# HuiyangYu/TGSFilter

Hardware: AMD Instinct MI355X
Metric: filtered Gbases/sec (end-to-end, excl. gzip I/O) (higher is better)
Workload: dtype u8

## Files before the change

include/tgsf_text.h:

```cpp
#ifndef TGSF_TEXT_H
#define TGSF_TEXT_H

#include "tgsf.h"

#ifdef __cplusplus
extern "C" {
#endif

#define TGSF_TEXT_ABI_VERSION 1
#define TGSF_TEXT_PAD 64u

enum {
    TGSF_TEXT_END = 0,
    TGSF_TEXT_IRREGULAR = 1,
    TGSF_TEXT_CAPACITY = 2
};

typedef struct tgsf_text_summary {
    uint32_t n_records;
    uint32_t stop;
    uint64_t consumed;
    uint64_t bases;
    uint32_t longest;
    float    device_ms;
} tgsf_text_summary;

typedef struct tgsf_text_index_arrays {
    uint64_t* seq_off;
    uint64_t* qual_off;
    uint32_t* len;
    uint64_t* name_off;
    uint32_t* name_len;
} tgsf_text_index_arrays;

typedef struct tgsf_text_device_buffers {
    uint8_t* text;
    tgsf_text_index_arrays index;
    tgsf_text_summary* summary;
    uint64_t max_bytes;
    uint32_t max_records;
    uint32_t reserved;
} tgsf_text_device_buffers;

typedef struct tgsf_text tgsf_text;

int tgsf_text_abi_version(void);
const char* tgsf_text_backend(void);

int tgsf_text_create(int device, uint64_t max_bytes, uint32_t max_records, tgsf_text** out);
void tgsf_text_destroy(tgsf_text* tx);
const char* tgsf_text_last_error(tgsf_text* tx);
int tgsf_text_profile(tgsf_text* tx, int enable);
int tgsf_text_buffers(tgsf_text* tx, tgsf_text_device_buffers* out);

int tgsf_text_index(tgsf_text* tx, const uint8_t* text, uint64_t n_bytes, int fasta, int final,
                    const tgsf_text_index_arrays* out_index, tgsf_text_summary* out_summary);

int tgsf_text_upload(tgsf_text* tx, const uint8_t* text, uint64_t n_bytes);

int tgsf_text_index_device(tgsf_text* tx, const uint8_t* d_text, uint64_t n_bytes, int fasta, int final,
                           const tgsf_text_index_arrays* d_index, tgsf_text_summary* d_summary, void* hip_stream);

int tgsf_text_fetch(tgsf_text* tx, const tgsf_text_index_arrays* out_index, tgsf_text_summary* out_summary);

int tgsf_text_submit(tgsf_text* tx, tgsf_ctx* ctx, const uint8_t* text, uint64_t n_bytes, int fasta, int final,
                     const tgsf_text_index_arrays* out_index, tgsf_text_summary* out_summary, tgsf_batch_out* batch_out);

#ifdef __cplusplus
}
#endif
#endif
```

tgsfilter_amd/csrc/tgsf_text.hip:

```cpp
#include <stdarg.h>
#include <stdio.h>
#include <stdlib.h>
#include <string.h>

#include <algorithm>
#include <string>
#include <vector>

#if defined(TGSF_EMUL)
#include "tgsf_text_kernels.h"
namespace tgsf_emul { thread_local Dim3 threadIdx, blockIdx, blockDim, gridDim; }
typedef void* rt_stream;
#include "tgsf_emul_rt.h"
#else
#include <hip/hip_runtime.h>
#include "tgsf_text_kernels.h"
typedef hipStream_t rt_stream;
static int rt_malloc(void** p, size_t n) { return (int)hipMalloc(p, n ? n : 1); }
static void rt_free(void* p) { (void)hipFree(p); }
static int rt_memset(void* p, int v, size_t n, rt_stream s) { return (int)hipMemsetAsync(p, v, n, s); }
static int rt_h2d(void* d, const void* s, size_t n, rt_stream st) { return (int)hipMemcpyAsync(d, s, n, hipMemcpyHostToDevice, st); }
static int rt_d2h(void* d, const void* s, size_t n, rt_stream st) { return (int)hipMemcpyAsync(d, s, n, hipMemcpyDeviceToHost, st); }
static int rt_sync(rt_stream s) { return (int)hipStreamSynchronize(s); }
static const char* rt_errstr(int e) { return hipGetErrorString((hipError_t)e); }
#define TGSF_LAUNCH(kernel, grid, block, stream, ...) hipLaunchKernelGGL(kernel, dim3(grid), dim3(block), 0, (stream), __VA_ARGS__)
#define TGSF_LAUNCH_COOP TGSF_LAUNCH
static unsigned grid_cap(unsigned g) { return g; }
#endif

using namespace tgsf;

static thread_local std::string g_create_error;

struct tgsf_text {
    int device;
    uint64_t max_bytes, max_pieces;
    uint32_t max_records;
    rt_stream stream;
    std::string error;
    bool profile = false;
    uint8_t* d_text = nullptr;
    uint64_t* d_bits = nullptr;
    uint32_t* d_cnt = nullptr;
    uint64_t* d_part = nullptr;
    uint64_t* d_table = nullptr;
    TextState* d_state = nullptr;
    tgsf_text_index_arrays d_index = {nullptr, nullptr, nullptr, nullptr, nullptr};
    tgsf_text_summary* d_summary = nullptr;
    tgsf_read_result* d_reads = nullptr;
    tgsf_fragment* d_frags = nullptr;
    uint32_t frag_cap = 0;
    uint32_t* d_nfrags = nullptr;
    std::vector<void*> allocs;
#if !defined(TGSF_EMUL)
    hipEvent_t ev[2] = {nullptr, nullptr};
    bool ev_recorded = false;
#endif
};

static int fail(tgsf_text* tx, int code, const char* fmt, ...)
{
    char buf[768];
    va_list ap;
    va_start(ap, fmt);
    vsnprintf(buf, sizeof buf, fmt, ap);
    va_end(ap);
    if (tx) tx->error = buf; else g_create_error = buf;
    return code;
}

template <class T>
static int dev_alloc(tgsf_text* tx, T** p, size_t count)
{
    void* q = nullptr;
    if (rt_malloc(&q, count * sizeof(T))) return 1;
    tx->allocs.push_back(q);
    *p = (T*)q;
    return 0;
}

extern "C" int tgsf_text_abi_version(void) { return TGSF_TEXT_ABI_VERSION; }
extern "C" const char* tgsf_text_backend(void) { return kTgsfEmul ? "emulation" : "hip:gfx950"; }
extern "C" const char* tgsf_text_last_error(tgsf_text* tx) { return tx ? tx->error.c_str() : g_create_error.c_str(); }

extern "C" void tgsf_text_destroy(tgsf_text* tx)
{
    if (!tx) return;
#if !defined(TGSF_EMUL)
    (void)hipSetDevice(tx->device);
    if (tx->stream) { (void)hipStreamSynchronize(tx->stream); (void)hipStreamDestroy(tx->stream); }
    for (hipEvent_t e : tx->ev) if (e) (void)hipEventDestroy(e);
#endif
    for (void* p : tx->allocs) rt_free(p);
    delete tx;
}

extern "C" int tgsf_text_create(int device, uint64_t max_bytes, uint32_t max_records, tgsf_text** out)
{
    if (!out) return fail(nullptr, TGSF_E_INVALID, "null argument");
    *out = nullptr;
    if (max_bytes == 0 || max_records == 0) return fail(nullptr, TGSF_E_INVALID, "max_bytes and max_records must be positive");
    const char* be = tgsf_backend();
    if (strncmp(be, kTgsfEmul ? "emulation" : "hip", kTgsfEmul ? 9 : 3) != 0)
        return fail(nullptr, TGSF_E_INVALID, "libtgsf_text (%s) is linked against the '%s' build of libtgsf", tgsf_text_backend(), be);
    tgsf_text* tx = new tgsf_text;
    tx->device = device;
    tx->max_bytes = max_bytes;
    tx->max_records = max_records;
    tx->max_pieces = (max_bytes + kTextPiece - 1) / kTextPiece;
    tx->stream = nullptr;
#if !defined(TGSF_EMUL)
    if (hipSetDevice(device) != hipSuccess) { delete tx; return fail(nullptr, TGSF_E_NO_DEVICE, "hipSetDevice(%d) failed: no usable HIP device (there is no CPU fallback)", device); }
    if (hipStreamCreateWithFlags(&tx->stream, hipStreamNonBlocking) != hipSuccess) { delete tx; return fail(nullptr, TGSF_E_HIP, "stream creation failed"); }
    for (hipEvent_t& e : tx->ev) if (hipEventCreate(&e) != hipSuccess) { tgsf_text_destroy(tx); return fail(nullptr, TGSF_E_HIP, "event creation failed"); }
#endif
    const uint64_t text_bytes = ((max_bytes + 15u) & ~15ull) + TGSF_TEXT_PAD;
    int e = 0;
    e |= dev_alloc(tx, &tx->d_text, text_bytes);
    if (!e) e |= dev_alloc(tx, &tx->d_bits, tx->max_pieces * kTextPieceWords);
    if (!e) e |= dev_alloc(tx, &tx->d_cnt, tx->max_pieces + 1);
    if (!e) e |= dev_alloc(tx, &tx->d_part, tx->max_pieces / kTextScanTile + 2);
    if (!e) e |= dev_alloc(tx, &tx->d_table, 4ull * max_records);
    if (!e) e |= dev_alloc(tx, &tx->d_state, 1);
    if (!e) e |= dev_alloc(tx, &tx->d_index.seq_off, max_records);
    if (!e) e |= dev_alloc(tx, &tx->d_index.qual_off, max_records);
    if (!e) e |= dev_alloc(tx, &tx->d_index.len, max_records);
    if (!e) e |= dev_alloc(tx, &tx->d_index.name_off, max_records);
    if (!e) e |= dev_alloc(tx, &tx->d_index.name_len, max_records);
    if (!e) e |= dev_alloc(tx, &tx->d_summary, 1);
    if (!e) e |= dev_alloc(tx, &tx->d_reads, max_records);
    if (!e) e |= dev_alloc(tx, &tx->d_nfrags, 4);
    if (e) {
        tgsf_text_destroy(tx);
        return fail(nullptr, TGSF_E_HIP, "device allocation failed (%llu bytes of text, %u records)", (unsigned long long)max_bytes, max_records);
    }
    *out = tx;
    return TGSF_OK;
}

extern "C" int tgsf_text_profile(tgsf_text* tx, int enable)
{
    if (!tx) return TGSF_E_INVALID;
    tx->profile = enable != 0;
    return TGSF_OK;
}

extern "C" int tgsf_text_buffers(tgsf_text* tx, tgsf_text_device_buffers* out)
{
    if (!tx) return TGSF_E_INVALID;
    if (!out) return fail(tx, TGSF_E_INVALID, "null argument");
    out->text = tx->d_text;
    out->index = tx->d_index;
    out->summary = tx->d_summary;
    out->max_bytes = tx->max_bytes;
    out->max_records = tx->max_records;
    out->reserved = 0;
    return TGSF_OK;
}

static unsigned blocks_for(uint64_t items, unsigned per_block) { return (unsigned)((items + per_block - 1) / per_block); }

static int enqueue_index(tgsf_text* tx, const uint8_t* d_text, uint64_t n, int fasta, int final,
                         const tgsf_text_index_arrays& I, tgsf_text_summary* d_summary, rt_stream st)
{
    const uint64_t pieces = (n + kTextPiece - 1) / kTextPiece;
    const uint32_t nb = (uint32_t)((pieces + kTextScanTile - 1) / kTextScanTile);
    const uint64_t cap = (fasta ? 2ull : 4ull) * tx->max_records;
    const unsigned gwave = blocks_for(pieces * kTextLanes, kTextThreads);
    const unsigned gemit = blocks_for((pieces + kTextEmitPieces - 1) / kTextEmitPieces * kTextLanes, kTextThreads);
    const unsigned gsmall = grid_cap(std::min(blocks_for(tx->max_records, kTextThreads), 2048u));
    const unsigned gfold = std::min(gsmall, 64u);
#if !defined(TGSF_EMUL)
    if (tx->profile) { (void)hipEventRecord(tx->ev[0], st); }
#endif
    if (pieces) {
        TGSF_LAUNCH(k_text_mark, gwave, kTextThreads, st, d_text, n, pieces, (uint16_t*)tx->d_bits, tx->d_cnt);
        TGSF_LAUNCH_COOP(k_text_scan_tiles, nb, 256, st, tx->d_cnt, pieces, tx->d_part);
    }
    TGSF_LAUNCH_COOP(k_text_scan_top, 1, 64, st, tx->d_part, nb, tx->d_state);
    if (pieces)
        TGSF_LAUNCH(k_text_emit, gemit, kTextThreads, st, (const uint64_t*)tx->d_bits, (const uint32_t*)tx->d_cnt,
                    (const uint64_t*)tx->d_part, pieces, tx->d_table, cap);
    TGSF_LAUNCH(k_text_check, gsmall, kTextThreads, st, d_text, n, fasta, final, (const uint64_t*)tx->d_table, tx->max_records, tx->d_state, I);
    TGSF_LAUNCH(k_text_fold, gfold, kTextThreads, st, (const uint32_t*)I.len, fasta, tx->max_records, tx->d_state);
    TGSF_LAUNCH_COOP(k_text_finish, 1, 64, st, n, fasta, final, (const uint64_t*)tx->d_table, tx->max_records, (const TextState*)tx->d_state, d_summary);
#if !defined(TGSF_EMUL)
    if (tx->profile) { (void)hipEventRecord(tx->ev[1], st); tx->ev_recorded = true; }
    if (hipGetLastError() != hipSuccess) return fail(tx, TGSF_E_HIP, "kernel launch failed");
#endif
    return TGSF_OK;
}

static float index_ms(tgsf_text* tx)
{
#if !defined(TGSF_EMUL)
    float ms = 0.0f;
    if (tx->profile && tx->ev_recorded && hipEventElapsedTime(&ms, tx->ev[0], tx->ev[1]) == hipSuccess) { tx->ev_recorded = false; return ms; }
    (void)hipGetLastError();
#endif
    (void)tx;
    return 0.0f;
}

static int check_args(tgsf_text* tx, uint64_t n_bytes, int fasta, int final)
{
    if ((fasta != 0 && fasta != 1) || (final != 0 && final != 1)) return fail(tx, TGSF_E_INVALID, "fasta and final are 0 or 1");
    if (n_bytes > tx->max_bytes)
        return fail(tx, TGSF_E_CAPACITY, "text of %llu bytes, the indexer was created for %llu", (unsigned long long)n_bytes, (unsigned long long)tx->max_bytes);
    return TGSF_OK;
}

static int upload(tgsf_text* tx, const uint8_t* text, uint64_t n_bytes)
{
    int he = 0;
    if (n_bytes) he |= rt_h2d(tx->d_text, text, n_bytes, tx->stream);
    he |= rt_memset(tx->d_text + n_bytes, 0, (size_t)((((n_bytes + 15u) & ~15ull) - n_bytes) + TGSF_TEXT_PAD), tx->stream);
    return he ? fail(tx, TGSF_E_HIP, "host to device copy failed: %s", rt_errstr(he)) : TGSF_OK;
}

extern "C" int tgsf_text_upload(tgsf_text* tx, const uint8_t* text, uint64_t n_bytes)
{
    if (!tx) return TGSF_E_INVALID;
    if (!text && n_bytes) return fail(tx, TGSF_E_INVALID, "null text");
    if (n_bytes > tx->max_bytes)
        return fail(tx, TGSF_E_CAPACITY, "text of %llu bytes, the indexer was created for %llu", (unsigned long long)n_bytes, (unsigned long long)tx->max_bytes);
#if !defined(TGSF_EMUL)
    (void)hipSetDevice(tx->device);
#endif
    int e = upload(tx, text, n_bytes);
    if (e) return e;
    const int he = rt_sync(tx->stream);
    return he ? fail(tx, TGSF_E_HIP, "stream synchronize failed: %s", rt_errstr(he)) : TGSF_OK;
}

extern "C" int tgsf_text_index_device(tgsf_text* tx, const uint8_t* d_text, uint64_t n_bytes, int fasta, int final,
                                      const tgsf_text_index_arrays* d_index, tgsf_text_summary* d_summary, void* hip_stream)
{
    if (!tx) return TGSF_E_INVALID;
    int e = check_args(tx, n_bytes, fasta, final);
    if (e) return e;
    if (!d_text) d_text = tx->d_text;
    if ((uintptr_t)d_text & 15u) return fail(tx, TGSF_E_INVALID, "the device text must be 16-byte aligned");
    if (d_index && (!d_index->seq_off || !d_index->qual_off || !d_index->len || !d_index->name_off || !d_index->name_len))
        return fail(tx, TGSF_E_INVALID, "a device index needs all five arrays");
#if !defined(TGSF_EMUL)
    (void)hipSetDevice(tx->device);
#endif
    return enqueue_index(tx, d_text, n_bytes, fasta, final, d_index ? *d_index : tx->d_index, d_summary ? d_summary : tx->d_summary,
                         hip_stream ? (rt_stream)hip_stream : tx->stream);
}

static int fetch(tgsf_text* tx, const tgsf_text_index_arrays* out_index, tgsf_text_summary* out_summary, tgsf_text_summary* sum)
{
    int he = rt_d2h(sum, tx->d_summary, sizeof *sum, tx->stream);
    if (!he) he = rt_sync(tx->stream);
    if (he) return fail(tx, TGSF_E_HIP, "device to host copy failed: %s", rt_errstr(he));
    sum->device_ms = index_ms(tx);
    const size_t k = sum->n_records;
    if (out_index && k) {
        if (out_index->seq_off) he |= rt_d2h(out_index->seq_off, tx->d_index.seq_off, k * 8, tx->stream);
        if (out_index->qual_off) he |= rt_d2h(out_index->qual_off, tx->d_index.qual_off, k * 8, tx->stream);
        if (out_index->len) he |= rt_d2h(out_index->len, tx->d_index.len, k * 4, tx->stream);
        if (out_index->name_off) he |= rt_d2h(out_index->name_off, tx->d_index.name_off, k * 8, tx->stream);
        if (out_index->name_len) he |= rt_d2h(out_index->name_len, tx->d_index.name_len, k * 4, tx->stream);
        if (!he) he = rt_sync(tx->stream);
        if (he) return fail(tx, TGSF_E_HIP, "device to host copy failed: %s", rt_errstr(he));
    }
    if (out_summary) *out_summary = *sum;
    return TGSF_OK;
}

extern "C" int tgsf_text_fetch(tgsf_text* tx, const tgsf_text_index_arrays* out_index, tgsf_text_summary* out_summary)
{
    if (!tx) return TGSF_E_INVALID;
#if !defined(TGSF_EMUL)
    (void)hipSetDevice(tx->device);
#endif
    tgsf_text_summary sum;
    return fetch(tx, out_index, out_summary, &sum);
}

extern "C" int tgsf_text_index(tgsf_text* tx, const uint8_t* text, uint64_t n_bytes, int fasta, int final,
                               const tgsf_text_index_arrays* out_index, tgsf_text_summary* out_summary)
{
    if (!tx) return TGSF_E_INVALID;
    if (!out_summary || (!text && n_bytes)) return fail(tx, TGSF_E_INVALID, "null argument");
    int e = check_args(tx, n_bytes, fasta, final);
    if (e) return e;
#if !defined(TGSF_EMUL)
    (void)hipSetDevice(tx->device);
#endif
    if ((e = upload(tx, text, n_bytes))) return e;
    if ((e = enqueue_index(tx, tx->d_text, n_bytes, fasta, final, tx->d_index, tx->d_summary, tx->stream))) return e;
    tgsf_text_summary sum;
    return fetch(tx, out_index, out_summary, &sum);
}

extern "C" int tgsf_text_submit(tgsf_text* tx, tgsf_ctx* ctx, const uint8_t* text, uint64_t n_bytes, int fasta, int final,
                                const tgsf_text_index_arrays* out_index, tgsf_text_summary* out_summary, tgsf_batch_out* bo)
{
    if (!tx) return TGSF_E_INVALID;
    if (!ctx || !out_summary || !bo || !bo->reads || (!text && n_bytes)) return fail(tx, TGSF_E_INVALID, "null argument");
    int e = check_args(tx, n_bytes, fasta, final);
    if (e) return e;
#if !defined(TGSF_EMUL)
    (void)hipSetDevice(tx->device);
#endif
    if (bo->frags && bo->frag_capacity > tx->frag_cap) {
        tgsf_fragment* f = nullptr;
        if (dev_alloc(tx, &f, bo->frag_capacity)) return fail(tx, TGSF_E_HIP, "device allocation failed (%u fragment records)", bo->frag_capacity);
        tx->d_frags = f;
        tx->frag_cap = bo->frag_capacity;
    }
    if ((e = upload(tx, text, n_bytes))) return e;
    if ((e = enqueue_index(tx, tx->d_text, n_bytes, fasta, final, tx->d_index, tx->d_summary, tx->stream))) return e;
    tgsf_text_summary sum;
    if ((e = fetch(tx, nullptr, nullptr, &sum))) return e;
    bo->n_frags = 0;
    if (sum.n_records) {
        tgsf_batch_in in;
        memset(&in, 0, sizeof in);
        in.seq = tx->d_text;
        in.qual = tx->d_text;
        in.offsets = tx->d_index.seq_off;
        in.lengths = tx->d_index.len;
        in.qual_offsets = tx->d_index.qual_off;
        in.n_reads = sum.n_records;
        in.n_bytes = n_bytes;
        tgsf_batch_out dout;
        dout.reads = tx->d_reads;
        dout.frags = bo->frags ? tx->d_frags : nullptr;
        dout.frag_capacity = bo->frags ? bo->frag_capacity : 0u;
        dout.n_frags = 0;
        e = tgsf_submit_device(ctx, &in, &dout, tx->d_nfrags, (void*)tx->stream);
        if (!e) e = tgsf_wait(ctx);
        if (e) return fail(tx, e, "libtgsf: %s", tgsf_last_error(ctx));
        uint32_t nf = 0;
        int he = rt_d2h(&nf, tx->d_nfrags, 4, tx->stream);
        he |= rt_d2h(bo->reads, tx->d_reads, (size_t)sum.n_records * sizeof(tgsf_read_result), tx->stream);
        if (!he) he = rt_sync(tx->stream);
        if (!he && nf > dout.frag_capacity) return fail(tx, TGSF_E_CAPACITY, "batch produced %u fragments, caller provided room for %u", nf, dout.frag_capacity);
        if (!he && nf) {
            he = rt_d2h(bo->frags, tx->d_frags, (size_t)nf * sizeof(tgsf_fragment), tx->stream);
            if (!he) he = rt_sync(tx->stream);
        }
        if (he) return fail(tx, TGSF_E_HIP, "device to host copy failed: %s", rt_errstr(he));
        bo->n_frags = nf;
    }
    tgsf_text_summary again;
    if (out_index && (e = fetch(tx, out_index, nullptr, &again))) return e;
    *out_summary = sum;
    return TGSF_OK;
}
```

tgsfilter_amd/host/api.cpp:

```cpp
#include "api.h"
#include "cputime.h"
#include "fatal.h"

#include <dlfcn.h>
#include <unistd.h>

#include <chrono>
#include <cstdio>
#include <cstdlib>
#include <iostream>
#include <string>
#include <thread>

#ifndef TGSF_LIB_REL
#define TGSF_LIB_REL "../libtgsf.so"
#endif
#ifndef TGSF_EXPECT_BACKEND
#define TGSF_EXPECT_BACKEND "hip"
#endif

namespace host {

namespace {
Api g_api;
std::thread g_thread;
std::string g_error;
double g_load_s = 0, g_device_s = 0;
bool g_started = false;

double now_s() { return std::chrono::duration<double>(std::chrono::steady_clock::now().time_since_epoch()).count(); }

std::string lib_path()
{
    if (const char* e = getenv("TGSF_LIB")) return e;
    char exe[4096];
    const ssize_t n = readlink("/proc/self/exe", exe, sizeof exe - 1);
    std::string dir = n > 0 ? std::string(exe, (size_t)n) : std::string(".");
    const size_t slash = dir.rfind('/');
    dir = slash == std::string::npos ? "." : dir.substr(0, slash);
    return dir + "/" + TGSF_LIB_REL;
}

void load(std::vector<int> devices)
{
    CpuScope cpu(CPU_LOADER);
    const double t0 = now_s();
    const std::string path = lib_path();
    void* h = dlopen(path.c_str(), RTLD_NOW | RTLD_LOCAL);
    if (!h) { g_error = std::string("cannot load ") + path + ": " + dlerror() + " (there is no CPU fallback)"; return; }
#define BIND(field, sym) \
    g_api.field = reinterpret_cast<decltype(g_api.field)>(dlsym(h, sym)); \
    if (!g_api.field) { g_error = std::string("symbol ") + sym + " missing in " + path; return; }
    BIND(abi_version, "tgsf_abi_version")
    BIND(backend, "tgsf_backend")
    BIND(prepare_device, "tgsf_prepare_device")
    BIND(create, "tgsf_create")
    BIND(destroy, "tgsf_destroy")
    BIND(submit, "tgsf_submit")
    BIND(wait, "tgsf_wait")
    BIND(counters_len, "tgsf_counters_len")
    BIND(counters, "tgsf_counters")
    BIND(counters_used, "tgsf_counters_used")
    BIND(align_windows, "tgsf_align_windows")
    BIND(last_error, "tgsf_last_error")
    BIND(profile, "tgsf_profile")
    BIND(stage_times, "tgsf_stage_times")
    BIND(stage_name, "tgsf_stage_name")
    BIND(device_location, "tgsf_device_location")
    BIND(counters_merge, "tgsf_counters_merge")
#undef BIND
    if (g_api.abi_version() != TGSF_ABI_VERSION) { g_error = path + ": ABI version mismatch"; return; }
    {
        const char* b = g_api.backend();
        const std::string want = TGSF_EXPECT_BACKEND;
        if (!b || std::string(b).compare(0, want.size(), want) != 0) {
            g_error = path + " is the \"" + (b ? b : "?") + "\" build of the library; this program runs on the \"" + want +
                      "\" build only (there is no CPU fallback; is TGSF_LIB set by accident?)";
            return;
        }
    }
    g_load_s = now_s() - t0;
    std::vector<std::thread> up;
    for (size_t i = 1; i < devices.size(); i++) {
        bool seen = false;
        for (size_t j = 0; j < i; j++) seen = seen || devices[j] == devices[i];
        if (!seen) up.emplace_back([d = devices[i]] { CpuScope c2(CPU_LOADER); (void)g_api.prepare_device(d); });
    }
    if (!devices.empty()) (void)g_api.prepare_device(devices[0]);
    for (std::thread& t : up) t.join();
    g_device_s = now_s() - t0 - g_load_s;
}
}

void lib_start(const std::vector<int>& devices)
{
    g_started = true;
    g_thread = std::thread(load, devices);
}

const Api& lib()
{
    if (!g_started) lib_start({});
    if (g_thread.joinable()) g_thread.join();
    if (!g_error.empty()) {
        std::cerr << "Error: " << g_error << std::endl;
        quit(255);
    }
    return g_api;
}

namespace {
RcclApi g_rccl;
bool g_rccl_ok = false, g_rccl_started = false;
std::thread g_rccl_thread;

void load_rccl()
{
    std::string path = lib_path();
    const size_t slash = path.rfind('/');
    path = (slash == std::string::npos ? std::string(".") : path.substr(0, slash)) + "/libtgsf_rccl.so";
    void* h = dlopen(path.c_str(), RTLD_NOW | RTLD_LOCAL);
    if (!h) return;
#define BIND(field, sym) g_rccl.field = reinterpret_cast<decltype(g_rccl.field)>(dlsym(h, sym)); if (!g_rccl.field) return;
    BIND(unique_id, "tgsf_rccl_unique_id")
    BIND(comm_init, "tgsf_rccl_comm_init")
    BIND(comm_count, "tgsf_rccl_comm_count")
    BIND(comm_destroy, "tgsf_rccl_comm_destroy")
    BIND(allreduce_counters, "tgsf_rccl_allreduce_counters")
    BIND(last_error, "tgsf_rccl_last_error")
#undef BIND
    g_rccl_ok = true;
}
}

void rccl_start()
{
    if (g_rccl_started) return;
    g_rccl_started = true;
    g_rccl_thread = std::thread(load_rccl);
}

const RcclApi* rccl_lib()
{
    rccl_start();
    if (g_rccl_thread.joinable()) g_rccl_thread.join();
    return g_rccl_ok ? &g_rccl : nullptr;
}

void lib_times(double& load_s, double& device_s) { load_s = g_load_s; device_s = g_device_s; }

}
```

tgsfilter_amd/host/api.h:

```cpp
#pragma once
#include <vector>

#include "tgsf.h"
#include "tgsf_rccl.h"

namespace host {

struct Api {
    decltype(&tgsf_abi_version) abi_version;
    decltype(&tgsf_backend) backend;
    decltype(&tgsf_prepare_device) prepare_device;
    decltype(&tgsf_create) create;
    decltype(&tgsf_destroy) destroy;
    decltype(&tgsf_submit) submit;
    decltype(&tgsf_wait) wait;
    decltype(&tgsf_counters_len) counters_len;
    decltype(&tgsf_counters) counters;
    decltype(&tgsf_counters_used) counters_used;
    decltype(&tgsf_align_windows) align_windows;
    decltype(&tgsf_last_error) last_error;
    decltype(&tgsf_profile) profile;
    decltype(&tgsf_stage_times) stage_times;
    decltype(&tgsf_stage_name) stage_name;
    decltype(&tgsf_device_location) device_location;
    decltype(&tgsf_counters_merge) counters_merge;
};

struct RcclApi {
    decltype(&tgsf_rccl_unique_id) unique_id;
    decltype(&tgsf_rccl_comm_init) comm_init;
    decltype(&tgsf_rccl_comm_count) comm_count;
    decltype(&tgsf_rccl_comm_destroy) comm_destroy;
    decltype(&tgsf_rccl_allreduce_counters) allreduce_counters;
    decltype(&tgsf_rccl_last_error) last_error;
};
void rccl_start();
const RcclApi* rccl_lib();

void lib_start(const std::vector<int>& devices);
const Api& lib();
void lib_times(double& load_s, double& device_s);

}
```

tgsfilter_amd/host/main.cpp:

```cpp
#include "run.h"

#include <malloc.h>
#include <signal.h>
#include <sys/prctl.h>
#include <sys/wait.h>

using namespace host;

static int g_done_fd = -1;

namespace host {

bool detached() { return g_done_fd >= 0; }

int cpu_budget()
{
    int hw = (int)std::thread::hardware_concurrency();
    if (hw <= 0) hw = 1;
    if (FILE* f = fopen("/sys/fs/cgroup/cpu.max", "r")) {
        char q[64] = {0};
        long long per = 0;
        if (fscanf(f, "%63s %lld", q, &per) == 2 && strcmp(q, "max") != 0 && per > 0) {
            const long long quota = atoll(q);
            if (quota > 0) hw = (int)std::min<long long>(hw, std::max<long long>(1, (quota + per - 1) / per));
        }
        fclose(f);
    }
    return hw;
}

[[noreturn]] void leave(int code)
{
    fflush(nullptr);
    if (code != 0) if (void (*f)() = on_die().exchange(nullptr)) f();
    if (g_done_fd >= 0) {
        prctl(PR_SET_PDEATHSIG, 0);
        if (write(g_done_fd, &code, sizeof code) != (ssize_t)sizeof code) {  }
        close(0); close(1); close(2);
    }
    _exit(code);
}

}

static void work_in_a_child()
{
    const char* d = getenv("TGSF_DETACH");
    if (!d || !*d || *d == '0') return;
    int fds[2];
    if (pipe(fds) != 0) return;
    const pid_t pid = fork();
    if (pid < 0) { close(fds[0]); close(fds[1]); return; }
    if (pid > 0) {
        close(fds[1]);
        int code = 0;
        ssize_t n;
        do { n = read(fds[0], &code, sizeof code); } while (n < 0 && errno == EINTR);
        if (n == (ssize_t)sizeof code) _exit(code);
        int st = 0;
        while (waitpid(pid, &st, 0) < 0 && errno == EINTR) {}
        _exit(WIFEXITED(st) ? WEXITSTATUS(st) : 128 + WTERMSIG(st));
    }
    close(fds[0]);
    g_done_fd = fds[1];
    prctl(PR_SET_PDEATHSIG, SIGTERM);
}


class InfoFilter : public std::streambuf {
public:
    explicit InfoFilter(std::streambuf* to, bool drop_info = true) : to_(to), drop_info_(drop_info) {}
protected:
    int overflow(int c) override {
        std::lock_guard<std::mutex> g(m_);
        if (c == traits_type::eof()) { flush_line(); return to_->pubsync() == 0 ? 0 : c; }
        line_.push_back((char)c);
        if (c == '\n') flush_line();
        return c;
    }
    std::streamsize xsputn(const char* s, std::streamsize n) override {
        std::lock_guard<std::mutex> g(m_);
        for (std::streamsize i = 0; i < n; i++) { line_.push_back(s[i]); if (s[i] == '\n') flush_line(); }
        return n;
    }
    int sync() override { std::lock_guard<std::mutex> g(m_); flush_line(); return to_->pubsync(); }
private:
    void flush_line() {
        if (drop_info_ && !line_.empty() && line_.back() == '\n' && line_.compare(0, 5, "INFO:") == 0) { line_.clear(); return; }
        if (!line_.empty() && line_.back() == '\n') { to_->sputn(line_.data(), (std::streamsize)line_.size()); line_.clear(); }
    }
    std::streambuf* to_;
    bool drop_info_;
    std::string line_;
    std::mutex m_;
};

int main(int argc, char** argv)
{
    double t_epoch0;
    { struct timespec ts; clock_gettime(CLOCK_REALTIME, &ts); t_epoch0 = (double)ts.tv_sec + ts.tv_nsec * 1e-9; }
    {
        const int r = shard_rank_on_command_line(argc, argv);
        if (r >= 0) std::cerr.rdbuf(new InfoFilter(std::cerr.rdbuf(), r > 0));
    }
    setenv("TGSF_SYNC", "blocking", 0);
    Options o;
    if (parse_args(argc, argv, o)) return 1;
    Run run(o);
    run.t_epoch0 = t_epoch0;
    if (const int rc = run.set_up_ranks()) return rc;
    if (run.o.ranks >= 1) std::cerr.rdbuf(new InfoFilter(std::cerr.rdbuf(), run.link.rank > 0));
    if (!run.sharded) work_in_a_child();
    {
        struct sigaction sa;
        memset(&sa, 0, sizeof sa);
        sa.sa_handler = [](int sig) { if (void (*f)() = on_die().exchange(nullptr)) f(); _exit(128 + sig); };
        sigaction(SIGINT, &sa, nullptr);
        sigaction(SIGTERM, &sa, nullptr);
    }
    mallopt(M_MMAP_THRESHOLD, 1 << 30);
    mallopt(M_TRIM_THRESHOLD, -1);
    run.timing = getenv("TGSF_TIMING") != nullptr;
    run.t_start = now_s();
    if (const int rc = run.check_file_types()) return rc;
    run.open_input();
    run.open_output_early();
    run.prepass();
    run.make_contexts();
    run.filter_pass();
    run.downsample();
    run.sum_tallies();
    run.report();
    if (run.timing) run.timing_lines();
    leave(0);
}
```

tgsfilter_amd/host/pipeline.h:

```cpp
#pragma once
#include <dlfcn.h>
#include <fcntl.h>
#include <malloc.h>
#include <sys/mman.h>
#include <sys/stat.h>
#include <sys/uio.h>
#include <unistd.h>
#include <zlib.h>

#include <algorithm>
#include <atomic>
#include <chrono>
#include <cmath>
#include <condition_variable>
#include <cstdio>
#include <cstring>
#include <deque>
#include <fstream>
#include <functional>
#include <iostream>
#include <map>
#include <memory>
#include <mutex>
#include <thread>
#include <unordered_map>
#include <unordered_set>

#include "cputime.h"
#include "fatal.h"
#include "fastx.h"
#include "options.h"
#include "tgsf.h"
#include "textsource.h"

namespace host {

struct CleanRec {
    std::string_view name;
    int pass_num;
    const char* seq;
    const char* qual;
    uint32_t len;
};

struct Batch {
    const char* base = nullptr;
    uint64_t span = 0;
    std::vector<uint64_t> off, qoff;
    std::vector<uint32_t> len;
    std::vector<Rec> recs;
    std::vector<tgsf_read_result> res;
    std::vector<tgsf_fragment> frags;
    uint32_t n_frags = 0;
    uint64_t bases = 0;
    uint64_t id = 0;
    struct Emit { CleanRec rec; uint64_t at; };
    std::vector<Emit> em;
    std::shared_ptr<Chunk> hold;
    char* dst = nullptr;
    uint64_t out_bytes = 0;
    std::atomic<int> left{0};
    void reset() {
        base = nullptr; span = 0; off.clear(); qoff.clear(); len.clear(); recs.clear(); n_frags = 0; bases = 0; id = 0;
        em.clear(); hold.reset(); dst = nullptr; out_bytes = 0; left = 0;
    }
};

class BatchStore {
public:
    std::shared_ptr<Batch> get() {
        {
            std::lock_guard<std::mutex> l(m_);
            if (!free_.empty()) { std::shared_ptr<Batch> b = std::move(free_.back()); free_.pop_back(); return b; }
        }
        std::shared_ptr<Batch> b(new Batch);
        b->off.reserve(4096); b->qoff.reserve(4096); b->len.reserve(4096); b->recs.reserve(4096);
        return b;
    }
    void put(std::shared_ptr<Batch> b) {
        b->reset();
        std::lock_guard<std::mutex> l(m_);
        free_.push_back(std::move(b));
    }
private:
    std::mutex m_;
    std::vector<std::shared_ptr<Batch>> free_;
};

template <class T>
class Channel {
public:
    explicit Channel(size_t cap) : cap_(cap) {}
    void put(T v) {
        std::unique_lock<std::mutex> l(m_);
        not_full_.wait(l, [&] { return q_.size() < cap_; });
        q_.push_back(std::move(v));
        not_empty_.notify_one();
    }
    T get() {
        std::unique_lock<std::mutex> l(m_);
        not_empty_.wait(l, [&] { return !q_.empty(); });
        T v = std::move(q_.front());
        q_.pop_front();
        not_full_.notify_one();
        return v;
    }
private:
    std::mutex m_;
    std::condition_variable not_full_, not_empty_;
    std::deque<T> q_;
    size_t cap_;
};

inline void append_name(std::string& out, std::string_view raw, int number)
{
    if (number < 2) { out.append(raw); return; }
    const std::string add = ":" + std::to_string(number);
    size_t i = 0;
    while (i < raw.size() && !std::isspace((unsigned char)raw[i])) i++;
    out.append(raw.substr(0, i));
    out += add;
    out.append(raw.substr(i));
}

inline double now_s()
{
    return std::chrono::duration<double>(std::chrono::steady_clock::now().time_since_epoch()).count();
}


class Deflater {
public:
    static const Deflater& get() { static const Deflater d; return d; }
    bool ok() const { return alloc_ && compress_ && bound_ && free__; }
    void* alloc(int level) const { return alloc_(level); }
    size_t bound(void* c, size_t n) const { return bound_(c, n); }
    size_t compress(void* c, const void* in, size_t n, void* out, size_t room) const { return compress_(c, in, n, out, room); }
    void free_(void* c) const { free__(c); }
private:
    Deflater() {
        if (knob("TGSF_ZLIB_OUTPUT")) return;
        for (const char* name : {"libdeflate.so.0", "libdeflate.so"}) {
            void* h = dlopen(name, RTLD_NOW | RTLD_LOCAL);
            if (!h) continue;
            alloc_ = reinterpret_cast<void* (*)(int)>(dlsym(h, "libdeflate_alloc_compressor"));
            compress_ = reinterpret_cast<size_t (*)(void*, const void*, size_t, void*, size_t)>(dlsym(h, "libdeflate_gzip_compress"));
            bound_ = reinterpret_cast<size_t (*)(void*, size_t)>(dlsym(h, "libdeflate_gzip_compress_bound"));
            free__ = reinterpret_cast<void (*)(void*)>(dlsym(h, "libdeflate_free_compressor"));
            if (ok()) return;
        }
    }
    void* (*alloc_)(int) = nullptr;
    size_t (*compress_)(void*, const void*, size_t, void*, size_t) = nullptr;
    size_t (*bound_)(void*, size_t) = nullptr;
    void (*free__)(void*) = nullptr;
};

class Output {
public:
    bool open(const Options& o) {
        gz_ = o.out_gz;
        if (o.out_file.empty()) f_ = stdout;
        else f_ = fopen(o.out_file.c_str(), "wb");
        if (!f_) { std::cerr << "Error: Failed to open file: " << o.out_file << std::endl; return false; }
        if (gz_) {
            setvbuf(f_, nullptr, _IOFBF, 8 << 20);
            level_ = o.comp_level;
            gz_threads_ = std::max(1, std::min(o.n_thread, 32));
        } else {
            fflush(f_);
            fd_ = fileno(f_);
        }
        return true;
    }
    void piece(const char* p, size_t n) {
        if (!n) return;
        if (gz_) { gzbuf_.append(p, n); return; }
        iov_.push_back({const_cast<char*>(p), n});
        if (iov_.size() >= 1000) flush_iov();
    }
    void text(const std::string& t) {
        if (gz_) { gzbuf_ += t; return; }
        if (pool_.size() + t.size() > pool_.capacity()) flush_iov();
        const size_t o0 = pool_.size();
        pool_ += t;
        iov_.push_back({&pool_[o0], t.size()});
    }
    void end_record() {
        if (!gz_) return;
        ends_.push_back(gzbuf_.size());
        if (gzbuf_.size() >= (256u << 20)) flush_gz();
    }
    void flush_gz() {
        if (ends_.empty()) return;
        const size_t nrec = ends_.size();
        const int T = (int)std::min<size_t>((size_t)gz_threads_, nrec);
        std::vector<std::vector<char>> outv((size_t)T);
        std::vector<size_t> cut((size_t)T + 1, nrec);
        cut[0] = 0;
        for (int t = 1; t < T; t++) {
            const size_t target = gzbuf_.size() / (size_t)T * (size_t)t;
            cut[(size_t)t] = (size_t)(std::lower_bound(ends_.begin(), ends_.end(), target) - ends_.begin());
        }
        std::atomic<bool> bad{false};
        const Deflater& ld = Deflater::get();
        auto work = [&](int t) {
            std::vector<char>& o = outv[(size_t)t];
            if (ld.ok()) {
                void* cz = ld.alloc(level_);
                if (!cz) { bad = true; return; }
                for (size_t r = cut[(size_t)t]; r < cut[(size_t)t + 1]; r++) {
                    const size_t b = r ? ends_[r - 1] : 0, n = ends_[r] - b;
                    const size_t at = o.size(), room = ld.bound(cz, n);
                    o.resize(at + room);
                    const size_t got = ld.compress(cz, gzbuf_.data() + b, n, o.data() + at, room);
                    if (!got) bad = true;
                    o.resize(at + got);
                }
                ld.free_(cz);
                return;
            }
            z_stream z;
            memset(&z, 0, sizeof z);
            if (deflateInit2(&z, level_, Z_DEFLATED, 15 + 16, 8, Z_DEFAULT_STRATEGY) != Z_OK) { bad = true; return; }
            for (size_t r = cut[(size_t)t]; r < cut[(size_t)t + 1]; r++) {
                const size_t b = r ? ends_[r - 1] : 0, n = ends_[r] - b;
                deflateReset(&z);
                const size_t at = o.size(), room = deflateBound(&z, (uLong)n) + 64;
                o.resize(at + room);
                z.next_in = (Bytef*)(gzbuf_.data() + b); z.avail_in = (uInt)n;
                z.next_out = (Bytef*)(o.data() + at); z.avail_out = (uInt)room;
                if (deflate(&z, Z_FINISH) != Z_STREAM_END) bad = true;
                o.resize(at + room - z.avail_out);
            }
            deflateEnd(&z);
        };
        std::vector<std::thread> th;
        for (int t = 1; t < T; t++) th.emplace_back(work, t);
        work(0);
        for (std::thread& x : th) x.join();
        if (bad) die("compression failed");
        for (const auto& o : outv) if (!o.empty() && fwrite(o.data(), 1, o.size(), f_) != o.size()) die("write failed");
        gzbuf_.clear();
        ends_.clear();
    }
    void flush_iov() {
        if (gz_) { flush_gz(); return; }
        size_t i = 0;
        while (i < iov_.size()) {
            ssize_t w = writev(fd_, &iov_[i], (int)std::min<size_t>(iov_.size() - i, 1000));
            if (w < 0) die("write failed");
            size_t left = (size_t)w;
            while (i < iov_.size() && left >= iov_[i].iov_len) { left -= iov_[i].iov_len; i++; }
            if (left) { iov_[i].iov_base = (char*)iov_[i].iov_base + left; iov_[i].iov_len -= left; }
        }
        iov_.clear();
        pool_.clear();
    }
    void close() {
        flush_iov();
        if (f_ && f_ != stdout) fclose(f_); else if (f_) fflush(f_);
        f_ = nullptr;
    }
    Output() { pool_.reserve(1 << 16); }
private:
    FILE* f_ = nullptr;
    int fd_ = -1;
    bool gz_ = false;
    int level_ = 6, gz_threads_ = 1;
    std::string gzbuf_, pool_;
    std::vector<size_t> ends_;
    std::vector<iovec> iov_;
};

class MappedSink {
public:
    bool open(const std::string& path, uint64_t virt_bytes, bool only_new = false) {
        fd_ = ::open(path.c_str(), only_new ? (O_RDWR | O_CREAT | O_EXCL) : (O_RDWR | O_CREAT | O_TRUNC), 0644);
        if (fd_ < 0) return false;
        created_ = only_new;
        path_ = path;
        struct stat st;
        bool ok = fstat(fd_, &st) == 0 && S_ISREG(st.st_mode) && fallocate(fd_, 0, 0, 4096) == 0 && ftruncate(fd_, 0) == 0;
        if (ok) {
            cap_ = (virt_bytes + 4095) & ~uint64_t(4095);
            map_ = (char*)mmap(nullptr, cap_, PROT_READ | PROT_WRITE, MAP_SHARED, fd_, 0);
            ok = map_ != MAP_FAILED;
            if (ok) madvise(map_, cap_, MADV_SEQUENTIAL);
        }
        if (!ok) { ::close(fd_); fd_ = -1; if (created_) unlink(path_.c_str()); return false; }
        live() = this;
        on_die().store([] { if (MappedSink* s = live()) s->cut_back(); });
        return true;
    }
    void cut_back() {
        if (fd_ < 0) return;
        dead_.store(true);
        const uint64_t size = size_.load();
        if (created_ && size == 0) { unlink(path_.c_str()); return; }
        if (reserved_.load() > size && ftruncate(fd_, (off_t)size) != 0) {  }
    }
    uint64_t reserved() const { return reserved_.load(); }
    uint64_t planned() const { return size_.load(); }
    uint64_t capacity() const { return cap_; }
    bool reserve_to(uint64_t end, bool must = true) {
        const uint64_t have = reserved_.load();
        if (end <= have) return true;
        if (dead_.load()) return false;
        const double t0 = now_s();
        if (fallocate(fd_, 0, (off_t)have, (off_t)(end - have)) != 0) {
            if (must) die(std::string("cannot extend the output file: ") + strerror(errno));
            return false;
        }
        t_falloc += now_s() - t0;
        reserved_.store(end);
        if (dead_.load()) { cut_back(); return false; }
        return true;
    }
    void populate(uint64_t at, uint64_t n) {
        char* p = map_ + (at & ~uint64_t(4095));
        const size_t len = (size_t)(((at + n + 4095) & ~uint64_t(4095)) - (at & ~uint64_t(4095)));
        if (madvise(p, len, 23 ) != 0)
            for (size_t o = 0; o < len; o += 4096) { volatile char* q = p + o; *q = *q; }
    }
    char* place(uint64_t n) { char* p = map_ + size_.load(); size_.fetch_add(n); return p; }
    static void release(const char* p, size_t n) {
        const uintptr_t lo = ((uintptr_t)p + 4095) & ~uintptr_t(4095), hi = ((uintptr_t)p + n) & ~uintptr_t(4095);
        if (hi > lo) madvise((void*)lo, hi - lo, MADV_DONTNEED);
    }
    void close() {
        if (fd_ < 0) return;
        if (reserved_.load() != size_.load() && ftruncate(fd_, (off_t)size_.load()) != 0) die("cannot set the size of the output file");
        ::close(fd_);
        fd_ = -1;
        if (live() == this) { live() = nullptr; on_die().store(nullptr); }
    }
    bool is_open() const { return fd_ >= 0; }
    double t_falloc = 0;
private:
    static MappedSink*& live() { static MappedSink* s = nullptr; return s; }
    int fd_ = -1;
    char* map_ = nullptr;
    std::atomic<uint64_t> size_{0}, reserved_{0};
    std::atomic<bool> dead_{false};
    uint64_t cap_ = 0;
    bool created_ = false;
    std::string path_;
};

#if defined(__x86_64__)
#include <immintrin.h>
__attribute__((target("avx2"))) inline void stream_copy_avx2(char* d, const char* s, size_t n)
{
    const size_t head = (size_t)(-(uintptr_t)d & 31u) < n ? (size_t)(-(uintptr_t)d & 31u) : n;
    memcpy(d, s, head);
    d += head; s += head; n -= head;
    size_t i = 0;
    for (; i + 128 <= n; i += 128) {
        const __m256i a = _mm256_loadu_si256((const __m256i*)(s + i)), b = _mm256_loadu_si256((const __m256i*)(s + i + 32));
        const __m256i c = _mm256_loadu_si256((const __m256i*)(s + i + 64)), e = _mm256_loadu_si256((const __m256i*)(s + i + 96));
        _mm256_stream_si256((__m256i*)(d + i), a); _mm256_stream_si256((__m256i*)(d + i + 32), b);
        _mm256_stream_si256((__m256i*)(d + i + 64), c); _mm256_stream_si256((__m256i*)(d + i + 96), e);
    }
    memcpy(d + i, s + i, n - i);
}
inline void stream_copy(char* d, const char* s, size_t n)
{
    static const bool avx2 = __builtin_cpu_supports("avx2");
    if (avx2 && n >= 4096) stream_copy_avx2(d, s, n); else memcpy(d, s, n);
}
inline void stream_fence() { _mm_sfence(); }
#else
inline void stream_copy(char* d, const char* s, size_t n) { memcpy(d, s, n); }
inline void stream_fence() {}
#endif

class Pool {
public:
    explicit Pool(int n, int cpu_stage = CPU_FILL) : stage_(cpu_stage) { for (int i = 0; i < n; i++) th_.emplace_back([this] { run(); }); }
    double busy_s() { std::lock_guard<std::mutex> l(m_); return busy_; }
    void add(std::function<void()> f) {
        { std::lock_guard<std::mutex> l(m_); q_.push_back(std::move(f)); open_++; }
        cv_.notify_one();
    }
    void drain() {
        std::unique_lock<std::mutex> l(m_);
        idle_.wait(l, [&] { return open_ == 0; });
    }
    void finish() {
        { std::lock_guard<std::mutex> l(m_); stop_ = true; }
        cv_.notify_all();
        for (std::thread& t : th_) t.join();
        th_.clear();
    }
private:
    void run() {
        CpuScope cpu(stage_);
        for (;;) {
            std::function<void()> f;
            {
                std::unique_lock<std::mutex> l(m_);
                cv_.wait(l, [&] { return stop_ || !q_.empty(); });
                if (q_.empty()) return;
                f = std::move(q_.front());
                q_.pop_front();
            }
            const double t0 = now_s();
            f();
            const double dt = now_s() - t0;
            f = nullptr;
            const double dd = now_s() - t0 - dt;
            std::lock_guard<std::mutex> l(m_);
            busy_ += dt;
            destroy_ += dd;
            if (dt > longest_) longest_ = dt;
            jobs_++;
            if (first_ == 0) first_ = t0;
            last_ = std::max(last_, t0 + dt + dd);
            if (--open_ == 0) idle_.notify_all();
        }
    }
    double busy_ = 0;
    const int stage_;
public:
    double destroy_ = 0, longest_ = 0, first_ = 0, last_ = 0;
    size_t jobs_ = 0;
private:
    size_t open_ = 0;
    std::condition_variable idle_;
    std::mutex m_;
    std::condition_variable cv_;
    std::deque<std::function<void()>> q_;
    std::vector<std::thread> th_;
    bool stop_ = false;
};

class Reserver {
public:
    Reserver(MappedSink& sink, Pool& populate, uint64_t stride) : sink_(sink), pop_(populate), stride_(stride) {}
    ~Reserver() { finish(); }
    void start(uint64_t speculative_limit) {
        goal_ = speculative_limit;
        th_ = std::thread([this] { run(); });
    }
    void want(uint64_t estimate, uint64_t need) {
        std::lock_guard<std::mutex> l(m_);
        if (need > need_) need_ = need;
        goal_ = estimate > need_ ? estimate : need_;
        cv_.notify_all();
    }
    void wait_ready(uint64_t upto) {
        std::unique_lock<std::mutex> l(m_);
        ready_cv_.wait(l, [&] { return ready_ >= upto; });
    }
    void finish() {
        { std::lock_guard<std::mutex> l(m_); stop_ = true; }
        cv_.notify_all();
        if (th_.joinable()) th_.join();
    }
    double t_populate_wait = 0;
private:
    void piece_done(size_t k) {
        std::lock_guard<std::mutex> l(m_);
        done_[k] = 1;
        while (next_ < done_.size() && done_[next_]) { ready_ = ends_[next_]; next_++; }
        ready_cv_.notify_all();
    }
    void run() {
        CpuScope cpu(CPU_FALLOCATE);
        uint64_t at = 0;
        for (;;) {
            uint64_t goal, need;
            {
                std::unique_lock<std::mutex> l(m_);
                cv_.wait(l, [&] { return stop_ || goal_ > at; });
                if (stop_ && at >= need_) return;
                if (goal_ <= at) return;
                goal = stop_ ? need_ : goal_; need = need_;
            }
            uint64_t upto = std::min<uint64_t>(goal, at + stride_);
            if (upto < sink_.reserved()) upto = sink_.reserved();
            if (!sink_.reserve_to(upto, false)) {
                if (need > at) { upto = need; sink_.reserve_to(upto); }
                else { std::lock_guard<std::mutex> l(m_); goal_ = at; continue; }
            }
            const uint64_t lo = at & ~uint64_t(4095), piece = 32u << 20;
            const double d0 = now_s();
            for (uint64_t o = lo; o < upto; o += piece) {
                const uint64_t n = std::min<uint64_t>(piece, upto - o);
                size_t k;
                { std::lock_guard<std::mutex> l(m_); k = done_.size(); done_.push_back(0); ends_.push_back(o + n); }
                pop_.add([this, o, n, k] { sink_.populate(o, n); piece_done(k); });
            }
            pop_.drain();
            t_populate_wait += now_s() - d0;
            at = upto;
        }
    }
    MappedSink& sink_;
    Pool& pop_;
    const uint64_t stride_;
    std::mutex m_;
    std::condition_variable cv_, ready_cv_;
    uint64_t goal_ = 0, need_ = 0, ready_ = 0;
    std::vector<char> done_;
    std::vector<uint64_t> ends_;
    size_t next_ = 0;
    bool stop_ = false;
    std::thread th_;
};

class MappedWriter {
public:
    MappedSink sink;
    bool is_open() const { return sink.is_open(); }
    bool open(const std::string& path, uint64_t capacity, bool only_new = false) { return sink.open(path, capacity, only_new); }
    void reserve_early(uint64_t limit) {
        early_ = std::thread([this, limit] {
            CpuScope cpu(CPU_FALLOCATE);
            while (!early_stop_.load() && sink.reserved() < limit)
                if (!sink.reserve_to(std::min<uint64_t>(limit, sink.reserved() + (256u << 20)), false)) break;
        });
    }
    void start_reserving(int populate_threads, uint64_t stride, uint64_t speculative) {
        if (early_.joinable()) { early_stop_ = true; early_.join(); }
        populate_.reset(new Pool(is_open() ? populate_threads : 0, CPU_POPULATE));
        reserver_.reset(new Reserver(sink, *populate_, stride));
        if (is_open()) reserver_->start(speculative);
    }
    void start_filling(int fill_threads, uint64_t release_piece) {
        pool_.reset(new Pool(is_open() ? fill_threads : 1));
        releaser_ = std::thread([this, release_piece] {
            CpuScope cpu(CPU_RELEASER);
            for (;;) {
                const std::pair<const char*, uint64_t> r = to_release_.get();
                if (!r.first) break;
                for (uint64_t o = 0; o < r.second; o += release_piece) MappedSink::release(r.first + o, std::min<uint64_t>(release_piece, r.second - o));
            }
        });
    }
    char* claim(uint64_t n, uint64_t estimate) {
        const uint64_t end = sink.planned() + n;
        if (end > sink.capacity()) die("output more than four times the size of the input: larger than the space mapped for it (TGSF_WRITER=writev writes such a file)");
        reserver_->want(std::min<uint64_t>(std::max<uint64_t>(estimate, end), sink.capacity()), end);
        const double d0 = now_s();
        reserver_->wait_ready(end);
        t_claim_wait += now_s() - d0;
        return sink.place(n);
    }
    void fill(std::function<void()> job) { pool_->add(std::move(job)); }
    void release(const char* p, uint64_t n) { to_release_.put({p, n}); }
    void finish() {
        reserver_->finish();
        t_planned = now_s();
        pool_->finish();
        populate_->finish();
        to_release_.put({nullptr, 0});
        releaser_.join();
        t_fill_tail = now_s() - t_planned;
        sink.close();
        t_close = now_s() - t_planned - t_fill_tail;
    }
    Pool& pool() { return *pool_; }
    double t_populate_wait() const { return reserver_->t_populate_wait; }
    double t_claim_wait = 0;
    double t_planned = 0, t_fill_tail = 0, t_close = 0;
private:
    std::atomic<bool> early_stop_{false};
    std::thread early_, releaser_;
    std::unique_ptr<Pool> populate_, pool_;
    std::unique_ptr<Reserver> reserver_;
    Channel<std::pair<const char*, uint64_t>> to_release_{1 << 16};
};

}
```

tgsfilter_amd/host/run.h:

```cpp
#pragma once
#include <memory>

#include "api.h"
#include "pipeline.h"
#include "prepass.h"
#include "report.h"
#include "shard.h"

namespace host {

int cpu_budget();
[[noreturn]] void leave(int code);
bool detached();

struct Run {
    explicit Run(Options& opts) : o(opts) {}

    int set_up_ranks();
    int check_file_types();
    void open_input();
    void open_output_early();
    void prepass();
    void make_contexts();
    void filter_pass();
    void downsample();
    void sum_tallies();
    void report();
    void timing_lines();

    Options& o;
    RankLink link;
    bool shard_may_use_rccl = false;
    bool sharded = false;
    bool timing = false;
    double t_epoch0 = 0, t_start = 0;
    double t_prepass = 0, t_pipe = 0, t_parse = 0, t_gpu = 0, t_write = 0, t_widle = 0, t_first = 0;

    std::string html;
    bool fasta_in = false;
    InputBytes in;
    bool streaming = false;
    size_t chunk_bytes = 64u << 20;
    int scan_threads = 1;
    size_t text_off = 0, text_size = 0;
    const char* text = nullptr;
    std::unique_ptr<RecordIndex> records_p;
    std::unique_ptr<ChunkReader> open_stream();

    std::string out_path;
    bool plain_file_out() const;
    MappedWriter mapped;
    Output out;
    bool fastq_out = false, run_filter_pass = true;

    PrepassResult pp;
    std::vector<std::string> adapters;

    uint64_t batch_text = 0;
    uint32_t batch_reads = 1u << 16;
    const Api* api = nullptr;
    double t_load = 0, t_dev = 0, t_libwait = 0;
    const RcclApi* R = nullptr;
    struct RcclUp { std::atomic<int> done{0}; int rc = TGSF_OK; std::string err; void* comm = nullptr; };
    std::shared_ptr<RcclUp> rccl_state = std::make_shared<RcclUp>();
    std::thread rccl_up;
    bool use_rccl = false;
    bool ranks_own_gpus = false;
    tgsf_params p;
    std::vector<int> ctx_dev;
    std::vector<tgsf_ctx*> ctxs;
    double t_p0 = 0;

    std::unique_ptr<Channel<std::shared_ptr<Batch>>> to_gpu, to_writer;
    std::vector<int> raw_lens, clean_lens;
    uint64_t raw_bases = 0, clean_bases = 0;
    uint64_t own_raw_bases = 0;
    std::vector<CleanRec> clean_recs;
    BatchStore store;
    std::atomic<uint64_t> stream_text{0};
    std::atomic<double> stream_share{0.0};
    std::mutex gpu_time_m;
    bool numa_bind = false;
    std::vector<int> dev_node;
    std::vector<double> dev_submit_s;
    std::vector<uint64_t> dev_bytes, dev_batches;
    int fill_threads = 1, populate_threads = 1;
    uint64_t fill_min = 1u << 20, stride_bytes = 2ull << 30;
    bool release_input = false, release_output = false;
    bool mapped_out = false;
    void reader_body();
    void feed(size_t k);
    void bind_to_node_of(size_t k);
    void writer_body();
    void fill_job(const std::shared_ptr<Batch>& b, size_t lo, size_t hi);
    void batch_done(std::shared_ptr<Batch> b);

    MappedWriter down_mapped;
    bool open_down_mapped(uint64_t capacity, uint64_t speculative);
    uint64_t down_bases = 0, down_job_recs = 0, down_job_bases = 0;
    std::vector<int> down_lens;
    std::vector<uint64_t> down_t;
    double t_dsel = 0, t_dcreate = 0, t_dqc = 0, t_dwrite = 0, t_dclose = 0, t_dsubmit = 0, t_dfirst = 0, d_kept = 0, d_span = 0;
    int n_dsubmit = 0;
    bool d_in_place = false, d_mapped = false;
    std::vector<char> select_kept();
    void second_pass(const std::vector<char>& keep);
    std::thread start_qc_feed(const std::vector<char>& keep, tgsf_ctx*& qctx, tgsf_ctx*& qctx2);
    void feed_in_place(const std::vector<uint32_t>& by_addr, const tgsf_params& qp, uint64_t kept_span, tgsf_ctx* qctx, tgsf_ctx*& qctx2);
    void feed_packed(const std::vector<char>& keep, const tgsf_params& qp, size_t room, tgsf_ctx* qctx);
    void write_kept(const std::vector<char>& keep);
    void merge_down_tallies(tgsf_ctx* qctx, tgsf_ctx* qctx2);

    uint64_t nw = 0;
    int32_t bc = 0;
    uint32_t nbins = 0;
    std::vector<uint64_t> t;
    double t_x0 = 0, t_rccl_wait = 0, t_allreduce = 0;
    int rccl_ranks = 0;
    std::string tally_route;
    bool reports() const { return !sharded || link.rank == 0; }
};

void add_tallies(std::vector<uint64_t>& v, const std::vector<uint64_t>& part, int32_t bc, uint32_t nbins);
std::vector<uint64_t> pack_rows(const std::vector<uint64_t>& v, int32_t bc, uint32_t nbins);
void add_rows(std::vector<uint64_t>& v, const std::vector<uint64_t>& ru, int32_t bc, uint32_t nbins);

}
```

tgsfilter_amd/host/run_contexts.cpp:

```cpp
#include "run.h"

namespace host {

void Run::prepass()
{
    std::unique_ptr<CpuScope> cpu_prepass(new CpuScope(CPU_PREPASS));
    if (sharded && link.rank > 0) {
    } else if (streaming) {
        std::unique_ptr<ChunkReader> cr = open_stream();
        std::shared_ptr<Chunk> ch;
        size_t at = 0;
        bool over = false;
        pp = run_prepass(o, [&](Rec& r) {
            while (!over && (!ch || at >= ch->recs.size())) {
                if (ch && !ch->message.empty()) std::cerr << ch->message << std::endl;
                if (ch && ch->last) { over = true; break; }
                ch = cr->next(o.in_file);
                at = 0;
                if (!ch) over = true;
            }
            if (over) return false;
            r = ch->recs[at++];
            return true;
        });
    } else if (sharded && link.world > 1) {
        RecordIndex whole(in.data(), in.size(), !fasta_in, std::max(scan_threads, std::min(8, cpu_budget() / 2)), 1u << 14);
        RecordIndex::Cursor cur(whole);
        pp = run_prepass(o, [&](Rec& r) { return cur.next(r); });
    } else {
        RecordIndex::Cursor cur(*records_p);
        pp = run_prepass(o, [&](Rec& r) { return cur.next(r); });
    }
    if (sharded) {
        BlobOut b;
        if (link.rank == 0) { b.pod(pp.qtype); b.pod(pp.trim5p); b.pod(pp.trim3p); b.pod(pp.depth5p); b.pod(pp.depth3p); b.pod(o.min_q); b.str(pp.adapter5p); b.str(pp.adapter3p); }
        link.bcast(b.s);
        BlobIn r(b.s);
        r.pod(pp.qtype); r.pod(pp.trim5p); r.pod(pp.trim3p); r.pod(pp.depth5p); r.pod(pp.depth3p); r.pod(o.min_q); r.str(pp.adapter5p); r.str(pp.adapter3p);
    }
    cpu_prepass.reset();
    t_prepass = now_s() - t_start;
    if (o.filter) {
        if (o.head_trim < 0) o.head_trim = pp.trim5p;
        if (o.tail_trim < 0) o.tail_trim = pp.trim3p;
        std::cerr << "INFO: trim 5' end length: " << o.head_trim << std::endl;
        std::cerr << "INFO: trim 3' end length: " << o.tail_trim << std::endl;
        std::cerr << "INFO: min output reads length: " << o.min_len << std::endl;
        if (!fasta_in) std::cerr << "INFO: min Phred average quality score: " << o.min_q << std::endl;
        auto add = [&](const std::string& a) { if (std::find(adapters.begin(), adapters.end(), a) == adapters.end()) adapters.push_back(a); };
        if (!o.adapter_file.empty()) {
            InputBytes af;
            if (af.open(o.adapter_file)) {
                const int ft = file_type(o.adapter_file);
                FastxReader rd(af.data(), af.size(), ft == 1);
                Record r;
                while (rd.next(r)) { add(std::string(r.seq)); add(rev_comp(std::string(r.seq))); }
            }
            int num = 0;
            for (const std::string& a : adapters) std::cerr << "INFO: input adapter " << ++num << " :" << a << std::endl;
        } else {
            std::string a5 = pp.adapter5p, a3 = pp.adapter3p;
            float d5 = pp.depth5p, d3 = pp.depth3p;
            if (d5 > 5 * d3) { a3.clear(); d3 = 0; } else if (d3 > 5 * d5) { a5.clear(); d5 = 0; }
            std::cerr << "INFO: 5' adapter: " << a5 << std::endl;
            std::cerr << "INFO: 3' adapter: " << a3 << std::endl;
            std::cerr << "INFO: mean depth of 5' adapter: " << d5 << std::endl;
            std::cerr << "INFO: mean depth of 3' adapter: " << d3 << std::endl;
            if (o.only_adapters) leave(0);
            if (!a5.empty()) { add(a5); add(rev_comp(a5)); }
            if (!a3.empty()) { add(a3); add(rev_comp(a3)); }
            if (a5.empty() && a3.empty()) {
                if (o.read_type == "hifi" || o.read_type == "clr") {
                    add(kAdapterLib[0]); add(kAdapterLib[1]);
                    std::cerr << "INFO: set PacBio blunt adapter to trim: " << kAdapterLib[0] << std::endl;
                } else if (o.read_type == "ont") {
                    add(kAdapterLib[8]); add(kAdapterLib[9]);
                    std::cerr << "INFO: set NanoPore rapid adapter to trim: " << kAdapterLib[8] << std::endl;
                }
            }
        }
    }
}

void Run::make_contexts()
{
    batch_text = streaming ? std::min<uint64_t>(256ull << 20, chunk_bytes)
                                    : std::min<uint64_t>(256ull << 20, std::max<uint64_t>(text_size / 8 + 4096, 1 << 16));
    if (const char* e = knob("TGSF_BATCH_BYTES")) { const long long v = atoll(e); if (v > 0) batch_text = (uint64_t)v; }
    batch_reads = 1u << 16;
    {
        uint64_t per_read = 0, cols = 0, words = 1;
        for (const std::string& a : adapters) {
            const int Q = (int)a.size();
            const int kmax = std::max(0, std::min(Q - 1, std::max(Q - o.end_match_len + 1, Q - o.mid_match_len + 1)));
            cols = std::max<uint64_t>(cols, (uint64_t)(Q + kmax + 2));
            words = std::max<uint64_t>(words, Q > 256 ? (uint64_t)(Q + 63) / 64 : Q > 128 ? 4 : Q > 64 ? 2 : 1);
        }
        per_read = cols * 2 * words * 8;
        if (words > 4) per_read = std::min<uint64_t>(per_read, (1ull << 20) + 16 * words) + 32 * words + 512;
        per_read *= 3 * std::max<size_t>(adapters.size(), 1);
        if (per_read) batch_reads = (uint32_t)std::min<uint64_t>(batch_reads, std::max<uint64_t>(256, (4ull << 30) / per_read));
    }
    fastq_out = o.out_type == 1;
    run_filter_pass = o.filter || o.only_qc;
    {
        const bool may_map = plain_file_out() && !o.only_qc && !o.downsample && run_filter_pass;
        if (may_map && !mapped.is_open()) mapped.open(out_path, streaming ? std::max<uint64_t>(64ull << 30, 64ull * in.size())
                                                                      : 4 * (uint64_t)text_size + (1ull << 30));
        Options oo = o;
        oo.out_file = out_path;
        if (!o.only_qc && !mapped.is_open() && !out.open(oo)) leave(1);
    }
    api = &lib();
    const Api& L = *api;
    lib_times(t_load, t_dev);
    t_libwait = now_s() - t_start - t_prepass;
    if (sharded) {
        const char* ex = getenv("TGSF_SHARD_EXCHANGE");
        if (shard_may_use_rccl) R = rccl_lib();
        char bus[64] = {0};
        int node = -1;
        if (L.device_location(o.device, bus, (int)sizeof bus, &node) != TGSF_OK) snprintf(bus, sizeof bus, "device%d", o.device);
        BlobOut mine;
        mine.str(bus);
        mine.pod<int>(R ? 1 : 0);
        const std::vector<std::string> all = link.gather(mine.s);
        std::string verdict(2, '0');
        if (link.rank == 0) {
            std::vector<std::string> seen;
            bool ok = R != nullptr, own = true;
            for (const std::string& a : all) {
                BlobIn in2(a);
                std::string b2; int have = 0;
                in2.str(b2); in2.pod(have);
                own = own && std::find(seen.begin(), seen.end(), b2) == seen.end();
                ok = ok && have;
                seen.push_back(b2);
            }
            ok = ok && own;
            verdict[0] = own ? '1' : '0';
            if (ok) {
                char id[TGSF_RCCL_ID_BYTES];
                if (R->unique_id(id) == TGSF_OK) { verdict[1] = '1'; verdict.append(id, sizeof id); }
                else if (ex && !strcmp(ex, "rccl")) die(std::string("TGSF_SHARD_EXCHANGE=rccl: ") + R->last_error());
            } else if (ex && !strcmp(ex, "rccl")) die("TGSF_SHARD_EXCHANGE=rccl: ranks share a GPU, or libtgsf_rccl.so does not load on every rank");
        }
        link.bcast(verdict);
        ranks_own_gpus = verdict.size() >= 2 && verdict[0] == '1';
        use_rccl = verdict.size() == 2 + TGSF_RCCL_ID_BYTES && verdict[1] == '1';
        if (use_rccl)
            rccl_up = std::thread([R = R, up = rccl_state, verdict, device = o.device, rank = link.rank, world = link.world] {
                if (const char* e = knob("TGSF_RCCL_STALL_S")) usleep((useconds_t)(atof(e) * 1e6));
                up->rc = R->comm_init(device, verdict.data() + 2, rank, world, &up->comm);
                if (up->rc != TGSF_OK) up->err = R->last_error();
                up->done.store(1, std::memory_order_release);
            });
    }
    memset(&p, 0, sizeof p);
    p.struct_size = sizeof p;
    p.min_len = o.min_len; p.max_len = o.max_len; p.min_q = o.min_q < 0 ? 0.f : o.min_q; p.max_q = o.max_q;
    p.bc_len = o.bc_len; p.head_trim = o.head_trim < 0 ? 0 : o.head_trim; p.tail_trim = o.tail_trim < 0 ? 0 : o.tail_trim;
    p.end_len = o.end_len; p.end_match_len = o.end_match_len; p.mid_match_len = o.mid_match_len; p.extra_len = o.extra_len;
    p.end_sim = o.end_sim; p.mid_sim = o.mid_sim; p.discard = o.discard; p.filter = o.filter; p.only_qc = o.only_qc;
    p.min_repeat = o.min_repeat; p.kmer = o.kmer; p.qtype = pp.qtype ? pp.qtype : 33;
    p.no_qual = fasta_in ? 1 : 0;
    if (adapters.size() > TGSF_MAX_ADAPTERS) die("more than " + std::to_string(TGSF_MAX_ADAPTERS) + " adapter sequences");
    p.n_adapters = (int)adapters.size();
    for (size_t a = 0; a < adapters.size(); a++) { p.adapters[a] = adapters[a].data(); p.adapter_len[a] = (int)adapters[a].size(); }
    p.max_batch_reads = batch_reads;
    if (streaming) p.max_read_len = 1u << 26;
    else if (sharded) {
        if (in.size() <= (1ull << 30)) { records_p->wait_complete(); p.max_read_len = (uint32_t)std::max<uint64_t>(link.max_u64(records_p->longest()), 1024); }
        else p.max_read_len = (uint32_t)std::min<uint64_t>(std::max<uint64_t>(in.size() / 2, 1024), 1u << 26);
    }
    else if (records_p->complete()) p.max_read_len = std::max<uint32_t>(records_p->longest(), 1024);
    else p.max_read_len = (uint32_t)std::min<uint64_t>(std::max<uint64_t>(in.size() / 2, 1024), 1u << 26);
    p.max_batch_bases = std::max<uint64_t>(batch_text, 2ull * p.max_read_len + (1u << 16)) + (1 << 20);
    int per_dev = (streaming || text_size > (64u << 20)) ? 3 : 1;
    if (const char* e = getenv("TGSF_CTX_PER_DEVICE")) { const int v = atoi(e); if (v >= 1 && v <= 8) per_dev = v; }
    for (int d : o.devices) for (int k = 0; k < per_dev; k++) ctx_dev.push_back(d);
    ctxs.assign(ctx_dev.size(), nullptr);
    t_p0 = now_s();
}

}
```

tgsfilter_amd/host/run_pipeline.cpp:

```cpp
#include "run.h"

#include <sched.h>

namespace host {

void Run::reader_body()
{
    CpuScope cpu(CPU_BATCHER);
    if (!run_filter_pass) { for (size_t d = 0; d < ctxs.size(); d++) to_gpu->put(nullptr); return; }
    std::unique_ptr<RecordIndex::Cursor> rd;
    if (!streaming) rd.reset(new RecordIndex::Cursor(*records_p));
    std::unique_ptr<ChunkReader> cr;
    if (streaming) cr = open_stream();
    std::shared_ptr<Chunk> ch;
    size_t ch_at = 0;
    bool over = false;
    Rec r;
    auto fresh = [&] { return store.get(); };
    std::shared_ptr<Batch> b = fresh();
    const double t0 = now_s();
    double waited = 0;
    uint64_t next_id = 0;
    auto flush = [&] {
        if (b->recs.empty()) return;
        const double w0 = now_s();
        b->id = next_id++;
        to_gpu->put(std::move(b));
        waited += now_s() - w0;
        b = fresh();
    };
    auto next_record = [&]() {
        if (!streaming) return rd->next(r);
        while (!over && (!ch || ch_at >= ch->recs.size())) {
            flush();
            if (ch && !ch->message.empty()) std::cerr << ch->message << std::endl;
            if (ch && ch->last) { over = true; break; }
            ch = cr->next(o.in_file);
            ch_at = 0;
            if (!ch) { over = true; break; }
            stream_text.store(cr->text_bytes());
            stream_share.store(cr->consumed());
        }
        if (over) return false;
        r = ch->recs[ch_at++];
        return true;
    };
    auto bad_cut = [&](size_t at) {
        die("--ranks / --shard: the input cannot be cut near byte " + std::to_string(at) + " the way one sequential reader would read it "
            "(lines the reader skips, or a malformed record, near there): run it without --ranks / --shard");
    };
    const char* last_end = nullptr;
    while (next_record()) {
        const size_t L = r.len;
        if (L > p.max_read_len) die("read longer than the supported maximum");
        const char* rec_end = (fasta_in ? r.seq : r.qual) + L;
        if (sharded && !last_end && link.rank > 0 && r.name != text + 1) bad_cut(text_off);
        last_end = rec_end;
        if (!b->recs.empty() && ((uint64_t)(rec_end - b->base) > batch_text || b->recs.size() >= batch_reads)) flush();
        if (b->recs.empty()) { b->base = r.name; b->hold = ch; }
        b->off.push_back((uint64_t)(r.seq - b->base));
        b->qoff.push_back(fasta_in ? b->off.back() : (uint64_t)(r.qual - b->base));
        b->len.push_back((uint32_t)L); b->recs.push_back(r);
        b->span = (uint64_t)(rec_end - b->base);
        if (b->span > p.max_batch_bases) die("record larger than a batch");
        b->bases += L;
        raw_bases += L; raw_lens.push_back((int)L);
    }
    if (sharded && link.rank + 1 < link.world) {
        const char* e = last_end ? last_end : text;
        const char* const end = text + text_size;
        if (e < end && *e == '\r') e++;
        if (e < end && *e == '\n') e++;
        if (e != end || !records_p->end_message().empty()) bad_cut(text_off + text_size);
    }
    flush();
    for (size_t d = 0; d < ctxs.size(); d++) to_gpu->put(nullptr);
    t_parse = now_s() - t0 - waited;
    std::sort(raw_lens.begin(), raw_lens.end());
}

void Run::bind_to_node_of(size_t k)
{
    const Api& L = *api;
    int node = -1;
    char bus[64];
    if (L.device_location(ctx_dev[k], bus, (int)sizeof bus, &node) == TGSF_OK && node >= 0) {
        const char* sysfs = knob("TGSF_SYSFS_NODES");
        std::ifstream f(std::string(sysfs ? sysfs : "/sys/devices/system/node") + "/node" + std::to_string(node) + "/cpulist");
        std::string list;
        cpu_set_t set;
        CPU_ZERO(&set);
        int n_set = 0;
        if (f && std::getline(f, list)) {
            size_t i = 0;
            while (i < list.size()) {
                const int a = atoi(list.c_str() + i);
                int b = a;
                size_t j = list.find_first_of(",-", i);
                if (j != std::string::npos && list[j] == '-') { b = atoi(list.c_str() + j + 1); j = list.find(',', j); }
                for (int c2 = a; c2 <= b && c2 < CPU_SETSIZE; c2++) { CPU_SET(c2, &set); n_set++; }
                i = j == std::string::npos ? list.size() : j + 1;
            }
        }
        cpu_set_t allowed;
        if (n_set > 0 && sched_getaffinity(0, sizeof allowed, &allowed) == 0) {
            n_set = 0;
            for (int c2 = 0; c2 < CPU_SETSIZE; c2++) {
                if (CPU_ISSET(c2, &set) && !CPU_ISSET(c2, &allowed)) CPU_CLR(c2, &set);
                if (CPU_ISSET(c2, &set)) n_set++;
            }
        }
        if (n_set > 0 && sched_setaffinity(0, sizeof set, &set) == 0) dev_node[k] = node;
    }
}

void Run::feed(size_t k)
{
    CpuScope cpu(CPU_FEEDER);
    const Api& L = *api;
    if (numa_bind) bind_to_node_of(k);
    if (L.create(&p, ctx_dev[k], &ctxs[k]) != TGSF_OK) die(L.last_error(nullptr));
    tgsf_ctx* fctx = ctxs[k];
    if (timing) (void)L.profile(fctx, 1);
    for (;;) {
        std::shared_ptr<Batch> b = to_gpu->get();
        if (!b) break;
        const double g0 = now_s();
        if (b->res.size() < b->recs.size()) b->res.resize(b->recs.size());
        const size_t fneed = (size_t)(b->bases / (uint64_t)std::max(p.min_len, 1)) + b->recs.size() + 16;
        if (b->frags.size() < fneed) b->frags.resize(fneed);
        const uint8_t* btext = reinterpret_cast<const uint8_t*>(b->base);
        tgsf_batch_in bi;
        memset(&bi, 0, sizeof bi);
        bi.seq = btext; bi.qual = btext;
        bi.offsets = b->off.data(); bi.qual_offsets = b->qoff.data(); bi.lengths = b->len.data();
        bi.n_reads = (uint32_t)b->recs.size(); bi.n_bytes = b->span;
        tgsf_batch_out bo{b->res.data(), b->frags.data(), (uint32_t)b->frags.size(), 0};
        if (L.submit(fctx, &bi, &bo) != TGSF_OK) die(L.last_error(fctx));
        { std::lock_guard<std::mutex> l(gpu_time_m); t_gpu += now_s() - g0; if (t_first == 0) t_first = now_s() - t_p0; }
        dev_submit_s[k] += now_s() - g0; dev_bytes[k] += b->span; dev_batches[k]++;
        b->n_frags = bo.n_frags;
        to_writer->put(std::move(b));
    }
    to_writer->put(nullptr);
}

void Run::batch_done(std::shared_ptr<Batch> b)
{
    if (b->out_bytes && release_output) mapped.release(b->dst, b->out_bytes);
    if (release_input) mapped.release(b->base, b->span);
    store.put(std::move(b));
}

void Run::filter_pass()
{
    to_gpu.reset(new Channel<std::shared_ptr<Batch>>(2 + ctxs.size()));
    to_writer.reset(new Channel<std::shared_ptr<Batch>>(256));
    if (!run_filter_pass) {
        RecordIndex::Cursor rd(*records_p);
        Rec r;
        while (rd.next(r)) {
            clean_recs.push_back({std::string_view(r.name, r.name_len), 1, r.seq, r.qual, r.len});
            clean_bases += r.len;
        }
    }

    std::thread reader([this] { reader_body(); });

    numa_bind = o.devices.size() > 1 || (link.world > 1 && ranks_own_gpus);
    if (const char* e = getenv("TGSF_NUMA")) numa_bind = atoi(e) > 0;
    dev_node.assign(ctx_dev.size(), -1);
    dev_submit_s.assign(ctx_dev.size(), 0.0);
    dev_bytes.assign(ctx_dev.size(), 0);
    dev_batches.assign(ctx_dev.size(), 0);
    std::vector<std::thread> feeders;
    for (size_t k = 0; k < ctxs.size(); k++) feeders.emplace_back([this, k] { feed(k); });

    fill_threads = std::max(1, std::min(o.n_thread, 16));
    fill_min = 1u << 20;
    if (const char* e = knob("TGSF_FILL_MIN_BYTES")) { const long long v = atoll(e); if (v > 0) fill_min = (uint64_t)v; }
    populate_threads = std::max(1, std::min(o.n_thread, 32));
    if (const char* e = knob("TGSF_POPULATE_THREADS")) { const int v = atoi(e); if (v >= 1 && v <= 64) populate_threads = v; }
    stride_bytes = streaming ? (128ull << 20) : (2ull << 30);
    if (const char* e = knob("TGSF_STRIDE_BYTES")) { const long long v = atoll(e); if (v > 0) stride_bytes = (uint64_t)v; }
    mapped.start_reserving(populate_threads, stride_bytes, (!streaming && text_size > (256u << 20)) ? (uint64_t)text_size / 4 : 0);
    {
        uint64_t early_min = 1ull << 30;
        if (const char* e = knob("TGSF_DOWN_EARLY_MIN")) early_min = strtoull(e, nullptr, 10);
        if (o.downsample && !streaming && in.mapped() && (uint64_t)text_size >= early_min) {
            uint64_t spec = (uint64_t)text_size / 4;
            if (o.genome_size > 0 && o.desired_depth > 0) spec = std::min<uint64_t>(spec, (2 * o.genome_size * (uint64_t)o.desired_depth) / (uint64_t)link.world + (uint64_t)text_size / 64);
            open_down_mapped(4 * (uint64_t)text_size + (1ull << 30), spec);
        }
    }
    const bool sync_exit = !detached();
    release_input = sync_exit && !streaming && in.mapped() && !o.downsample;
    release_output = sync_exit || streaming;
    mapped.start_filling(fill_threads, 16u << 20);
    std::thread writer([this] { writer_body(); });
    reader.join();
    for (std::thread& f : feeders) f.join();
    writer.join();
    mapped_out = mapped.is_open();
    mapped.finish();
    t_pipe = now_s() - t_p0;
}

}
```

tgsfilter_amd/host/run_report.cpp:

```cpp
#include "run.h"

#include <sys/stat.h>

namespace host {

std::vector<uint64_t> pack_rows(const std::vector<uint64_t>& v, int32_t bc2, uint32_t nb2)
{
    const size_t head = tgsf_ctr_bin_table(0, bc2, nb2);
    std::vector<uint64_t> out(v.begin(), v.begin() + (long)head);
    for (int b = 0; b < 4; b++) {
        const size_t at = tgsf_ctr_bin_table(b, bc2, nb2), n = (size_t)std::min<uint64_t>(v[TGSF_CTR_ROWS + (b >> 1)], nb2) * 5;
        out.insert(out.end(), v.begin() + (long)at, v.begin() + (long)(at + n));
    }
    return out;
}

void add_tallies(std::vector<uint64_t>& v, const std::vector<uint64_t>& part, int32_t bc2, uint32_t nb2)
{
    uint64_t rows[4];
    for (int q = 0; q < 4; q++) rows[q] = std::max(v[TGSF_CTR_ROWS + q], part[TGSF_CTR_ROWS + q]);
    const size_t head = tgsf_ctr_bin_table(0, bc2, nb2);
    for (size_t i = 0; i < head; i++) v[i] += part[i];
    for (int b = 0; b < 4; b++) {
        const size_t at = tgsf_ctr_bin_table(b, bc2, nb2), n = (size_t)std::min<uint64_t>(part[TGSF_CTR_ROWS + (b >> 1)], nb2) * 5;
        for (size_t i = 0; i < n; i++) v[at + i] += part[at + i];
    }
    for (int q = 0; q < 4; q++) v[TGSF_CTR_ROWS + q] = rows[q];
}

void add_rows(std::vector<uint64_t>& v, const std::vector<uint64_t>& ru, int32_t bc2, uint32_t nb2)
{
    const size_t head = tgsf_ctr_bin_table(0, bc2, nb2);
    if (ru.size() < head) die("a rank of the job sent a tally vector of another layout");
    std::vector<uint64_t> whole(v.size(), 0);
    std::copy(ru.begin(), ru.begin() + (long)head, whole.begin());
    size_t from = head;
    for (int b = 0; b < 4; b++) {
        const size_t at = tgsf_ctr_bin_table(b, bc2, nb2), n = (size_t)std::min<uint64_t>(ru[TGSF_CTR_ROWS + (b >> 1)], nb2) * 5;
        if (from + n > ru.size()) die("a rank of the job sent a tally vector of another layout");
        std::copy(ru.begin() + (long)from, ru.begin() + (long)(from + n), whole.begin() + (long)at);
        from += n;
    }
    add_tallies(v, whole, bc2, nb2);
}

static void add_context(const Api& L, tgsf_ctx* c, std::vector<uint64_t>& v, std::vector<uint64_t>& part, int32_t bc, uint32_t nbins)
{
    if (L.counters_used(c, part.data(), part.size(), nullptr) != TGSF_OK) die(L.last_error(c));
    add_tallies(v, part, bc, nbins);
}

void Run::sum_tallies()
{
    const Api& L = *api;
    tgsf_ctx* ctx = ctxs[0];
    void* rccl_comm = nullptr;
    int rccl_rc = TGSF_OK;
    std::string rccl_err;
    L.counters_len(ctx, &nw, &bc, &nbins);
    t.assign(nw, 0);
    std::vector<uint64_t> part(nw);
    t_x0 = now_s();
    own_raw_bases = raw_bases;
    const char* ex = getenv("TGSF_SHARD_EXCHANGE");
    const bool must_rccl = ex && !strcmp(ex, "rccl");
    for (tgsf_ctx* c : ctxs) add_context(L, c, t, part, bc, nbins);
    if (!sharded) return;

    if (use_rccl) {
        double rccl_patience = 120.0;
        if (const char* e = knob("TGSF_RCCL_INIT_TIMEOUT_S")) rccl_patience = atof(e);
        while (!rccl_state->done.load(std::memory_order_acquire) && now_s() - t_x0 < rccl_patience) usleep(2000);
        if (rccl_state->done.load(std::memory_order_acquire)) {
            rccl_up.join();
            rccl_rc = rccl_state->rc; rccl_err = rccl_state->err; rccl_comm = rccl_state->comm;
        } else {
            rccl_up.detach();
            rccl_rc = TGSF_E_HIP;
            rccl_err = "the communicator was not up " + std::to_string((int)rccl_patience) + " s after the filtering ended";
        }
        t_rccl_wait = now_s() - t_x0;
        if (link.max_u64(rccl_rc != TGSF_OK ? 1 : 0) != 0) {
            if (must_rccl) die("RCCL communicator: " + (rccl_err.empty() ? std::string("it failed on another rank") : rccl_err));
            if (rccl_rc != TGSF_OK) std::cerr << "Warning: rank " << link.rank << ": RCCL communicator: " << rccl_err << " -- the tallies are summed over the ranks' sockets" << std::endl;
            rccl_comm = nullptr;
            use_rccl = false;
        }
    }
    std::vector<uint64_t> reduced;
    if (use_rccl) {
        for (size_t k = 1; k < ctxs.size(); k++)
            if (L.counters_merge(ctxs[0], ctxs[k]) != TGSF_OK) die(L.last_error(ctxs[0]));
        struct Reduce { std::atomic<int> done{0}; int rc = TGSF_OK; std::string err; double s = 0; };
        const std::shared_ptr<Reduce> rd = std::make_shared<Reduce>();
        double patience = 60.0;
        if (const char* e = knob("TGSF_RCCL_ALLREDUCE_TIMEOUT_S")) patience = atof(e);
        const double a0 = now_s();
        std::thread helper([R = R, rd, c0 = ctxs[0], rccl_comm, rank = link.rank, world = link.world, a0] {
            if (const char* e = knob("TGSF_RCCL_ALLREDUCE_STALL_S")) usleep((useconds_t)(atof(e) * 1e6));
            rd->rc = R->allreduce_counters(c0, rccl_comm, rank, world, 0, nullptr);
            if (rd->rc != TGSF_OK) rd->err = R->last_error();
            rd->s = now_s() - a0;
            rd->done.store(1, std::memory_order_release);
        });
        while (!rd->done.load(std::memory_order_acquire) && now_s() - a0 < patience) usleep(500);
        int bad = 0;
        if (rd->done.load(std::memory_order_acquire)) {
            helper.join();
            t_allreduce = rd->s;
            if (rd->rc != TGSF_OK) { bad = 1; rccl_err = "tally all-reduce: " + rd->err; }
        } else {
            helper.detach();
            bad = 1;
            rccl_err = "the tally all-reduce had not returned after " + std::to_string((int)patience) + " s";
        }
        if (link.max_u64((uint64_t)bad) != 0) {
            if (must_rccl) die(rccl_err.empty() ? std::string("tally all-reduce: it failed on another rank") : rccl_err);
            if (bad) std::cerr << "Warning: rank " << link.rank << ": " << rccl_err << " -- the tallies summed over the ranks' sockets are used" << std::endl;
            use_rccl = false;
        } else {
            (void)R->comm_count(rccl_comm, &rccl_ranks);
            reduced.assign(nw, 0);
            add_context(L, ctxs[0], reduced, part, bc, nbins);
        }
    }
    BlobOut mine;
    mine.pod(raw_bases); mine.pod(clean_bases);
    mine.vec(raw_lens); mine.vec(clean_lens);
    mine.vec(pack_rows(t, bc, nbins));
    const std::vector<std::string> all = link.gather(mine.s);
    for (int k = 1; k < (int)all.size(); k++) {
        BlobIn in2(all[(size_t)k]);
        uint64_t rb = 0, cb = 0;
        std::vector<int> rl, cl;
        std::vector<uint64_t> ru;
        in2.pod(rb); in2.pod(cb); in2.vec(rl); in2.vec(cl); in2.vec(ru);
        raw_bases += rb; clean_bases += cb;
        const size_t r0 = raw_lens.size(), c0 = clean_lens.size();
        raw_lens.insert(raw_lens.end(), rl.begin(), rl.end());
        clean_lens.insert(clean_lens.end(), cl.begin(), cl.end());
        std::inplace_merge(raw_lens.begin(), raw_lens.begin() + (long)r0, raw_lens.end());
        if (!o.downsample) std::inplace_merge(clean_lens.begin(), clean_lens.begin() + (long)c0, clean_lens.end());
        add_rows(t, ru, bc, nbins);
    }
    tally_route = "summed on rank 0 over the ranks' sockets";
    if (use_rccl) {
        tally_route = "RCCL all-reduce on the devices";
        if (link.rank == 0) {
            if (pack_rows(reduced, bc, nbins) == pack_rows(t, bc, nbins)) { t.swap(reduced); tally_route += ", equal to the sum over the ranks' sockets"; }
            else {
                if (must_rccl) die("the all-reduced tally vector differs from the sum of the ranks' vectors over their sockets");
                std::cerr << "Warning: the all-reduced tally vector differs from the sum of the ranks' vectors over their sockets -- the sockets' sum is used" << std::endl;
                tally_route += " (DIFFERENT from the sum over the ranks' sockets, which is used)";
            }
        }
    }
    if (timing)
        fprintf(stderr, "SHARD %d/%d: bytes [%zu, %zu) of the text on device %d -> %s | tallies: %s (communicator ready after %.3f s of waiting, all-reduce %.4f s, %d ranks in it), exchange + gather %.3f s\n",
                link.rank, link.world, text_off, text_off + text_size, o.device, out_path.c_str(), tally_route.c_str(), t_rccl_wait, t_allreduce, rccl_ranks, now_s() - t_x0);
    if (use_rccl) R->comm_destroy(rccl_comm);
}

void Run::report()
{
    auto tables = [&](const std::vector<uint64_t>& v, bool clean) {
        SideTables s;
        s.bin_qual = &v[tgsf_ctr_bin_table(clean ? TGSF_B_CLEAN_QUAL : TGSF_B_RAW_QUAL, bc, nbins)];
        s.bin_cnt = &v[tgsf_ctr_bin_table(clean ? TGSF_B_CLEAN_CNT : TGSF_B_RAW_CNT, bc, nbins)];
        s.bin_rows = v[TGSF_CTR_ROWS + (clean ? 1 : 0)];
        s.q5 = &v[tgsf_ctr_end_table(clean ? TGSF_T_CLEAN5P_QUAL : TGSF_T_RAW5P_QUAL, bc)];
        s.c5 = &v[tgsf_ctr_end_table(clean ? TGSF_T_CLEAN5P_CNT : TGSF_T_RAW5P_CNT, bc)];
        s.q3 = &v[tgsf_ctr_end_table(clean ? TGSF_T_CLEAN3P_QUAL : TGSF_T_RAW3P_QUAL, bc)];
        s.c3 = &v[tgsf_ctr_end_table(clean ? TGSF_T_CLEAN3P_CNT : TGSF_T_RAW3P_CNT, bc)];
        s.end_rows = v[TGSF_CTR_ROWS + (clean ? 3 : 2)];
        s.diff_qual = &v[clean ? TGSF_CTR_CLEAN_DIFFQ : TGSF_CTR_RAW_DIFFQ];
        return s;
    };
    SideStats raw, clean;
    const int clean_num = (int)clean_lens.size();
    if (run_filter_pass && reports()) {
        if (raw_lens.empty()) die("no reads in the input");
        std::sort(raw_lens.begin(), raw_lens.end());
        side_stats(bc, raw_lens, raw_bases, tables(t, false), raw);
        if (!o.only_qc && !o.downsample) {
            if (clean_lens.empty()) die("no reads passed the filters");
            std::sort(clean_lens.begin(), clean_lens.end());
            side_stats(bc, clean_lens, clean_bases, tables(t, true), clean);
        }
        const uint64_t* d = &t[TGSF_CTR_DROPINFO];
        std::cerr << "INFO: " << raw_lens.size() << " reads with a total of " << raw_bases << " bases were input." << std::endl;
        if (!o.only_qc) {
            std::cerr << "INFO: " << d[0] << " reads were discarded with " << d[1] << " bases due to low quality." << std::endl;
            std::cerr << "INFO: " << d[2] << " reads have adapter at 5', 3' and middle." << std::endl;
            std::cerr << "INFO: " << d[3] << " reads have adapter at 5' and middle." << std::endl;
            std::cerr << "INFO: " << d[4] << " reads have adapter at 3' and middle." << std::endl;
            std::cerr << "INFO: " << d[5] << " reads have adapter at 5' and 3' end." << std::endl;
            std::cerr << "INFO: " << d[6] << " reads only have adapter at middle." << std::endl;
            std::cerr << "INFO: " << d[7] << " reads only have adapter at 5' end." << std::endl;
            std::cerr << "INFO: " << d[8] << " reads only have adapter at 3' end." << std::endl;
            std::cerr << "INFO: " << d[9] << " reads didn't have any adapter." << std::endl;
            std::cerr << "INFO: " << d[10] << " bases were trimmed due to the adapter or base content bias." << std::endl;
            std::cerr << "INFO: " << d[11] << " reads were discarded with " << d[12] << " bases due to the short length." << std::endl;
            std::cerr << "INFO: " << d[13] << " reads were discarded with " << d[14] << " bases due to low quality after split." << std::endl;
            if (o.min_repeat > 0)
                std::cerr << "INFO: " << d[15] << " reads were discarded with " << d[16] << " bases due to short repeat length." << std::endl;
            std::cerr << "INFO: " << clean_num << " reads with a total of " << clean_bases << " bases after filtering." << std::endl;
            if (!o.downsample && !o.out_file.empty()) {
                if (!sharded) std::cerr << "INFO: Filtered reads were written to: " << o.out_file << "." << std::endl;
                else std::cerr << "INFO: Filtered reads were written to: " << o.out_file << ".part0 ... " << o.out_file << ".part" << link.world - 1
                               << " (" << link.world << " parts; concatenated in this order they are the reads in input order)." << std::endl;
            }
        }
    }
    if (reports() && sharded && !o.out_file.empty() && !o.only_qc && !o.only_adapters) {
        const std::string list = o.out_file + ".parts";
        std::vector<std::string> earlier;
        {
            std::ifstream f(list);
            std::string line;
            if (f && std::getline(f, line) && line == "# tgsfilter parts, in order")
                while (std::getline(f, line)) if (!line.empty()) earlier.push_back(line);
        }
        std::vector<std::string> mine;
        for (int k = 0; k < link.world; k++) mine.push_back(o.out_file + ".part" + std::to_string(k));
        for (const std::string& e : earlier) {
            if (std::find(mine.begin(), mine.end(), e) != mine.end()) continue;
            const std::string stem = o.out_file + ".part";
            if (e.compare(0, stem.size(), stem) != 0 || e.size() == stem.size() || e.find_first_not_of("0123456789", stem.size()) != std::string::npos) continue;
            struct stat st;
            if (lstat(e.c_str(), &st) == 0 && S_ISREG(st.st_mode) && unlink(e.c_str()) == 0)
                std::cerr << "Warning: " << e << ", a part of an earlier job with more ranks, was removed." << std::endl;
        }
        for (int k = link.world; k < link.world + 1024; k++) {
            const std::string other = o.out_file + ".part" + std::to_string(k);
            struct stat st;
            if (lstat(other.c_str(), &st) != 0) { if (k >= link.world + 64) break; else continue; }
            std::cerr << "Warning: " << other << " exists and is not a part of this job (nor of an earlier one this tool listed): `cat " << o.out_file
                      << ".part*` would take it in -- the parts of this job are listed in " << list << "." << std::endl;
        }
        std::ofstream f(list, std::ios::trunc);
        f << "# tgsfilter parts, in order\n";
        for (const std::string& m : mine) f << m << "\n";
    }
    if (o.downsample && reports()) {
        if (down_lens.empty()) die("no reads to downsample");
        std::sort(down_lens.begin(), down_lens.end());
        side_stats(bc, down_lens, down_bases, tables(down_t, false), clean);
        clean.tab[8] = limit_decimals(std::round(clean.mean_qual * 1000) / 1000.0, 2);
        if (!o.filter)
            std::cerr << "INFO: " << (sharded ? down_job_recs : clean_recs.size()) << " reads with a total of " << (sharded ? down_job_bases : clean_bases) << " bases were input." << std::endl;
        std::cerr << "INFO: " << down_lens.size() << " reads with a total of " << down_bases << " bases after downsampling." << std::endl;
        if (!o.out_file.empty()) {
            if (!sharded) std::cerr << "INFO: Downsampled reads were written to: " << o.out_file << "." << std::endl;
            else std::cerr << "INFO: Downsampled reads were written to: " << o.out_file << ".part0 ... " << o.out_file << ".part" << link.world - 1
                           << " (" << link.world << " parts; concatenated in this order they are the reads in input order)." << std::endl;
        }
    }
    std::string qc = fasta_in ? "0" : "1";
    qc += o.only_qc ? "0" : ((!o.filter && o.downsample) ? "1" : "2");
    if (reports()) {
        std::ofstream ofs(html);
        write_report(ofs, qc, raw, clean);
        ofs.close();
        std::cerr << "INFO: Quality control report was written to: " << html << "." << std::endl;
    }
}

void Run::timing_lines()
{
    const Api& L = *api;
    if (timing) {
        Pool& fills = mapped.pool();
        const double t_busy = fills.busy_s();
        fprintf(stderr, "POOL: %zu jobs, busy %.3f, freeing job state %.3f, longest job %.3f, first job at %.3f, last job done at %.3f (pipeline start = 0, planner done at %.3f)\n",
                fills.jobs_, t_busy, fills.destroy_, fills.longest_, fills.first_ - t_p0, fills.last_ - t_p0, mapped.t_planned - t_p0);
        fprintf(stderr, "TIMING: total %.3f s | index+prepass %.3f | waiting for the library %.3f (load %.3f + device %.3f, beside the pre-pass) | "
                        "pipeline %.3f (batching %.3f, tgsf_submit summed over %zu feeders %.3f, plan+write %.3f, planner waiting %.3f, "
                        "first batch filtered after %.3f, fill tail %.3f, closing the output %.3f; stages overlap) | stats+report %.3f | %s (fallocate %.3f, mapping the reserved pages %.3f, fill threads busy %.3f summed)\n",
                now_s() - t_start, t_prepass, t_libwait, t_load, t_dev, t_pipe, t_parse, ctxs.size(), t_gpu, t_write, t_widle, t_first,
                mapped.t_fill_tail, mapped.t_close, now_s() - t_p0 - t_pipe, mapped_out ? "output: fallocate + mapped fill" : "output: writev", mapped.sink.t_falloc, mapped.t_populate_wait(), t_busy);
        fprintf(stderr, "RESERVE: planner waited %.3f s for pages of the output file\n", mapped.t_claim_wait);
    }
    if (timing) {
        float tot[TGSF_N_STAGES] = {0};
        uint32_t nb = 0;
        for (tgsf_ctx* c : ctxs) {
            float ms[TGSF_N_STAGES]; uint32_t n1 = 0;
            if (c && L.stage_times(c, ms, &n1) == TGSF_OK) { nb += n1; for (int i = 0; i < TGSF_N_STAGES; i++) tot[i] += ms[i]; }
        }
        double sum = 0;
        for (int i = 0; i < TGSF_N_STAGES; i++) sum += tot[i];
        char piece[256];
        snprintf(piece, sizeof piece, "GPU: kernels %.3f s summed over %zu contexts and %u batches (upper bound of the busy time: contexts overlap) = %.4f of the run |", sum * 1e-3, ctxs.size(), nb,
                 sum * 1e-3 / std::max(1e-9, now_s() - t_start));
        std::string line = piece;
        for (int i = 0; i < TGSF_N_STAGES; i++) if (tot[i] > 0) { snprintf(piece, sizeof piece, " %s %.1f ms", L.stage_name(i), tot[i]); line += piece; }
        line += "\n";
        fputs(line.c_str(), stderr);
    }
    if (timing) {
        for (size_t di = 0; di < o.devices.size(); di++) {
            if (std::find(o.devices.begin(), o.devices.begin() + (long)di, o.devices[di]) != o.devices.begin() + (long)di) continue;
            double sub = 0; uint64_t by = 0, nb2 = 0; int nf2 = 0, node = -1;
            for (size_t k = 0; k < ctx_dev.size(); k++)
                if (ctx_dev[k] == o.devices[di]) { sub += dev_submit_s[k]; by += dev_bytes[k]; nb2 += dev_batches[k]; nf2++; node = std::max(node, dev_node[k]); }
            fprintf(stderr, "DEVICE %d: %llu batches, %.2f GB of text through %d feeders, tgsf_submit %.3f s summed = %.1f GB/s per feeder, %.1f GB/s for the device over the pipeline's %.3f s%s\n",
                    o.devices[di], (unsigned long long)nb2, by * 1e-9, nf2, sub, sub > 0 ? by * 1e-9 / sub : 0.0, t_pipe > 0 ? by * 1e-9 / t_pipe : 0.0, t_pipe,
                    node >= 0 ? (" (feeders bound to NUMA node " + std::to_string(node) + ")").c_str() : "");
        }
    }
    if (timing) {
        const double proc = process_cpu_s();
        double own = 0;
        std::string line;
        char piece[160];
        for (int s = 0; s < CPU_N; s++) {
            double v = (double)cpu_ns()[s].load() * 1e-9;
            if (s == CPU_MAIN) v += (double)thread_cpu_ns() * 1e-9 - (double)cpu_ns()[CPU_PREPASS].load() * 1e-9;
            own += v;
            if (v >= 0.0005) { snprintf(piece, sizeof piece, "%s %s %.3f", line.empty() ? "" : ",", cpu_stage_name(s), v); line += piece; }
        }
        snprintf(piece, sizeof piece, "CPU: %.3f s of CPU time (user + system) for %.3f Gbases = %.4f CPU-s per Gbase |", proc, (double)own_raw_bases * 1e-9,
                 own_raw_bases ? proc / ((double)own_raw_bases * 1e-9) : 0.0);
        std::string head = piece;
        snprintf(piece, sizeof piece, " | threads of the runtime and others %.3f\n", proc - own);
        fputs((head + line + piece).c_str(), stderr);
    }
    if (timing && o.downsample)
        fprintf(stderr, "DOWN: selection %.3f | QC pass over the kept reads (%s, %.2f GB of them in %.2f GB of text): context %.3f, batches + submits %.3f (its own thread; %d submits %.3f, the first %.3f) | writing them %.3f (%s) | closing the output %.3f\n",
                t_dsel, d_in_place ? "read in place" : "packed", d_kept * 1e-9, d_span * 1e-9, t_dcreate, t_dqc, n_dsubmit, t_dsubmit, t_dfirst, t_dwrite, d_mapped ? "fallocate + threads into a mapping" : "writev", t_dclose);
    if (timing) {
        struct timespec ts; clock_gettime(CLOCK_REALTIME, &ts);
        fprintf(stderr, "CLOCK: main entered at %.6f, leaving at %.6f (epoch seconds)\n", t_epoch0, (double)ts.tv_sec + ts.tv_nsec * 1e-9);
    }
}

}
```

tgsfilter_amd/text.py:

```python
from __future__ import annotations

import ctypes as C
import os
from collections import namedtuple

import numpy as np

from . import abi
from .capi import TgsfError

_HERE = os.path.dirname(os.path.abspath(__file__))
DEFAULT_LIB = os.path.join(_HERE, "libtgsf_text.so")
_LIBS = {}

ABI_VERSION = 1
END, IRREGULAR, CAPACITY = 0, 1, 2
STOP_NAMES = {END: "END", IRREGULAR: "IRREGULAR", CAPACITY: "CAPACITY"}
PAD = 64

SYMBOLS = [
    "tgsf_text_abi_version", "tgsf_text_backend", "tgsf_text_create", "tgsf_text_destroy", "tgsf_text_last_error", "tgsf_text_profile",
    "tgsf_text_buffers", "tgsf_text_index", "tgsf_text_upload", "tgsf_text_index_device", "tgsf_text_fetch", "tgsf_text_submit",
]


class Summary(C.Structure):
    _fields_ = [("n_records", C.c_uint32), ("stop", C.c_uint32), ("consumed", C.c_uint64), ("bases", C.c_uint64),
                ("longest", C.c_uint32), ("device_ms", C.c_float)]

    def as_dict(self):
        return {"n_records": self.n_records, "stop": self.stop, "consumed": self.consumed, "bases": self.bases,
                "longest": self.longest, "device_ms": self.device_ms}


class IndexArrays(C.Structure):
    _fields_ = [("seq_off", C.c_void_p), ("qual_off", C.c_void_p), ("len", C.c_void_p), ("name_off", C.c_void_p), ("name_len", C.c_void_p)]


class DeviceBuffers(C.Structure):
    _fields_ = [("text", C.c_void_p), ("index", IndexArrays), ("summary", C.c_void_p), ("max_bytes", C.c_uint64),
                ("max_records", C.c_uint32), ("reserved", C.c_uint32)]


assert C.sizeof(Summary) == 32

Index = namedtuple("Index", "seq_off qual_off len name_off name_len")


def load(path: str | None = None):
    explicit = path is not None
    path = path or DEFAULT_LIB
    if path not in _LIBS:
        if not os.path.exists(path):
            raise FileNotFoundError(
                f"{path} not found: build the HIP extension first (python -c 'import __graft_entry__ as g; g.build()')")
        L = C.CDLL(path)
        vp, u64, i = C.c_void_p, C.c_uint64, C.c_int
        L.tgsf_text_abi_version.restype = i
        L.tgsf_text_backend.restype = C.c_char_p
        L.tgsf_text_create.argtypes = [i, u64, C.c_uint32, C.POINTER(vp)]
        L.tgsf_text_destroy.argtypes = [vp]
        L.tgsf_text_destroy.restype = None
        L.tgsf_text_last_error.argtypes = [vp]
        L.tgsf_text_last_error.restype = C.c_char_p
        L.tgsf_text_profile.argtypes = [vp, i]
        L.tgsf_text_buffers.argtypes = [vp, C.POINTER(DeviceBuffers)]
        L.tgsf_text_index.argtypes = [vp, vp, u64, i, i, C.POINTER(IndexArrays), C.POINTER(Summary)]
        L.tgsf_text_upload.argtypes = [vp, vp, u64]
        L.tgsf_text_index_device.argtypes = [vp, vp, u64, i, i, C.POINTER(IndexArrays), vp, vp]
        L.tgsf_text_fetch.argtypes = [vp, C.POINTER(IndexArrays), C.POINTER(Summary)]
        L.tgsf_text_submit.argtypes = [vp, vp, vp, u64, i, i, C.POINTER(IndexArrays), C.POINTER(Summary), C.POINTER(abi.BatchOut)]
        if L.tgsf_text_abi_version() != ABI_VERSION:
            raise RuntimeError("libtgsf_text ABI version mismatch")
        _LIBS[path] = L
    L = _LIBS[path]
    if not explicit and not L.tgsf_text_backend().startswith(b"hip"):
        raise RuntimeError(f"{path} is the {L.tgsf_text_backend().decode()!r} build of libtgsf_text, not the HIP build (there is no CPU fallback)")
    return L


def _as_u8(text):
    if isinstance(text, (bytes, bytearray, memoryview)):
        return np.frombuffer(text, dtype=np.uint8)
    return np.ascontiguousarray(text, dtype=np.uint8)


class TextIndexer:

    def __init__(self, device: int, max_bytes: int, max_records: int, lib_path: str | None = None):
        self.lib = load(lib_path)
        self.max_bytes, self.max_records = int(max_bytes), int(max_records)
        h = C.c_void_p()
        rc = self.lib.tgsf_text_create(device, self.max_bytes, self.max_records, C.byref(h))
        if rc != 0:
            raise TgsfError(rc, self.lib.tgsf_text_last_error(None).decode())
        self.h = h

    def _chk(self, rc):
        if rc != 0:
            raise TgsfError(rc, self.lib.tgsf_text_last_error(self.h).decode())

    def close(self):
        if getattr(self, "h", None):
            self.lib.tgsf_text_destroy(self.h)
            self.h = None

    def __del__(self):
        try:
            self.close()
        except Exception:
            pass

    def profile(self, enable=True):
        self._chk(self.lib.tgsf_text_profile(self.h, int(enable)))

    def buffers(self) -> DeviceBuffers:
        b = DeviceBuffers()
        self._chk(self.lib.tgsf_text_buffers(self.h, C.byref(b)))
        return b

    def _host_index(self):
        m = self.max_records
        arrs = Index(np.zeros(m, np.uint64), np.zeros(m, np.uint64), np.zeros(m, np.uint32), np.zeros(m, np.uint64), np.zeros(m, np.uint32))
        return arrs, IndexArrays(*[a.ctypes.data for a in arrs])

    @staticmethod
    def _clip(arrs, n):
        return Index(*[a[:n].copy() for a in arrs])

    def index(self, text, fasta=False, final=True):
        t = _as_u8(text)
        arrs, ia = self._host_index()
        s = Summary()
        self._chk(self.lib.tgsf_text_index(self.h, t.ctypes.data, t.size, int(fasta), int(final), C.byref(ia), C.byref(s)))
        return self._clip(arrs, s.n_records), s.as_dict()

    def upload(self, text):
        t = _as_u8(text)
        self._chk(self.lib.tgsf_text_upload(self.h, t.ctypes.data, t.size))
        return t.size

    def index_device(self, n_bytes, fasta=False, final=True, d_text=None, d_index: IndexArrays | None = None, d_summary=None, stream=None):
        self._chk(self.lib.tgsf_text_index_device(self.h, d_text, int(n_bytes), int(fasta), int(final),
                                                  C.byref(d_index) if d_index is not None else None, d_summary, stream))

    def fetch(self, want_index=True):
        s = Summary()
        if not want_index:
            self._chk(self.lib.tgsf_text_fetch(self.h, None, C.byref(s)))
            return None, s.as_dict()
        arrs, ia = self._host_index()
        self._chk(self.lib.tgsf_text_fetch(self.h, C.byref(ia), C.byref(s)))
        return self._clip(arrs, s.n_records), s.as_dict()

    def submit(self, ctx, text, fasta=False, final=True, frag_capacity=None, want_index=True):
        t = _as_u8(text)
        if frag_capacity is None:
            frag_capacity = t.size // 100 + self.max_records + 16
        arrs, ia = self._host_index() if want_index else (None, None)
        reads = np.zeros(self.max_records, dtype=abi.READ_RESULT_DTYPE)
        frags = np.zeros(frag_capacity, dtype=abi.FRAGMENT_DTYPE)
        bo = abi.BatchOut(reads.ctypes.data, frags.ctypes.data, frag_capacity, 0)
        s = Summary()
        self._chk(self.lib.tgsf_text_submit(self.h, ctx.h, t.ctypes.data, t.size, int(fasta), int(final),
                                            C.byref(ia) if want_index else None, C.byref(s), C.byref(bo)))
        n = s.n_records
        return (self._clip(arrs, n) if want_index else None), s.as_dict(), reads[:n].copy(), frags[:bo.n_frags].copy()
```

Baseline: 6.853.

## Upload batches to device-resident slots ahead of filtering via pinned staging

```diff
diff --git a/include/tgsf_text.h b/include/tgsf_text.h
--- a/include/tgsf_text.h
+++ b/include/tgsf_text.h
@@ -7,7 +7,7 @@
 extern "C" {
 #endif
 
-#define TGSF_TEXT_ABI_VERSION 1
+#define TGSF_TEXT_ABI_VERSION 2
 #define TGSF_TEXT_PAD 64u
 
 enum {
@@ -66,6 +66,12 @@
 int tgsf_text_submit(tgsf_text* tx, tgsf_ctx* ctx, const uint8_t* text, uint64_t n_bytes, int fasta, int final,
                      const tgsf_text_index_arrays* out_index, tgsf_text_summary* out_summary, tgsf_batch_out* batch_out);
 
+int tgsf_text_create_resident(int device, uint64_t max_bytes, uint32_t max_records, tgsf_text** out);
+int tgsf_text_upload_batch(tgsf_text* tx, tgsf_text* via, const uint8_t* text, uint64_t n_bytes,
+                           const uint64_t* seq_off, const uint64_t* qual_off, const uint32_t* len, uint32_t n_records);
+int tgsf_text_filter_resident(tgsf_text* tx, tgsf_ctx* ctx, tgsf_batch_out* batch_out);
+int tgsf_text_device_memory(int device, uint64_t* free_bytes, uint64_t* total_bytes);
+
 #ifdef __cplusplus
 }
 #endif
diff --git a/tgsfilter_amd/csrc/tgsf_text.hip b/tgsfilter_amd/csrc/tgsf_text.hip
--- a/tgsfilter_amd/csrc/tgsf_text.hip
+++ b/tgsfilter_amd/csrc/tgsf_text.hip
@@ -31,6 +31,12 @@
 using namespace tgsf;
 
 static thread_local std::string g_create_error;
+
+static const char* knob(const char* name)
+{
+    static const bool on = [] { const char* e = getenv("TGSF_DEBUG_KNOBS"); return e && e[0] == '1'; }();
+    return on ? getenv(name) : nullptr;
+}
 
 struct tgsf_text {
     int device;
@@ -52,9 +58,15 @@
     uint32_t frag_cap = 0;
     uint32_t* d_nfrags = nullptr;
     std::vector<void*> allocs;
+    bool resident_only = false;
+    uint64_t res_bytes = 0;
+    uint32_t res_records = 0;
 #if !defined(TGSF_EMUL)
     hipEvent_t ev[2] = {nullptr, nullptr};
     bool ev_recorded = false;
+    uint8_t* stage[2] = {nullptr, nullptr};
+    hipEvent_t stage_ev[2] = {nullptr, nullptr};
+    size_t stage_bytes = 0;
 #endif
 };
 
@@ -90,12 +102,14 @@
     (void)hipSetDevice(tx->device);
     if (tx->stream) { (void)hipStreamSynchronize(tx->stream); (void)hipStreamDestroy(tx->stream); }
     for (hipEvent_t e : tx->ev) if (e) (void)hipEventDestroy(e);
+    for (hipEvent_t e : tx->stage_ev) if (e) (void)hipEventDestroy(e);
+    for (uint8_t* b : tx->stage) if (b) (void)hipHostFree(b);
 #endif
     for (void* p : tx->allocs) rt_free(p);
     delete tx;
 }
 
-extern "C" int tgsf_text_create(int device, uint64_t max_bytes, uint32_t max_records, tgsf_text** out)
+static int create(int device, uint64_t max_bytes, uint32_t max_records, bool resident_only, tgsf_text** out)
 {
     if (!out) return fail(nullptr, TGSF_E_INVALID, "null argument");
     *out = nullptr;
@@ -104,6 +118,7 @@
     if (strncmp(be, kTgsfEmul ? "emulation" : "hip", kTgsfEmul ? 9 : 3) != 0)
         return fail(nullptr, TGSF_E_INVALID, "libtgsf_text (%s) is linked against the '%s' build of libtgsf", tgsf_text_backend(), be);
     tgsf_text* tx = new tgsf_text;
+    tx->resident_only = resident_only;
     tx->device = device;
     tx->max_bytes = max_bytes;
     tx->max_records = max_records;
@@ -116,26 +131,52 @@
 #endif
     const uint64_t text_bytes = ((max_bytes + 15u) & ~15ull) + TGSF_TEXT_PAD;
     int e = 0;
-    e |= dev_alloc(tx, &tx->d_text, text_bytes);
-    if (!e) e |= dev_alloc(tx, &tx->d_bits, tx->max_pieces * kTextPieceWords);
-    if (!e) e |= dev_alloc(tx, &tx->d_cnt, tx->max_pieces + 1);
-    if (!e) e |= dev_alloc(tx, &tx->d_part, tx->max_pieces / kTextScanTile + 2);
-    if (!e) e |= dev_alloc(tx, &tx->d_table, 4ull * max_records);
-    if (!e) e |= dev_alloc(tx, &tx->d_state, 1);
-    if (!e) e |= dev_alloc(tx, &tx->d_index.seq_off, max_records);
-    if (!e) e |= dev_alloc(tx, &tx->d_index.qual_off, max_records);
-    if (!e) e |= dev_alloc(tx, &tx->d_index.len, max_records);
-    if (!e) e |= dev_alloc(tx, &tx->d_index.name_off, max_records);
-    if (!e) e |= dev_alloc(tx, &tx->d_index.name_len, max_records);
-    if (!e) e |= dev_alloc(tx, &tx->d_summary, 1);
-    if (!e) e |= dev_alloc(tx, &tx->d_reads, max_records);
-    if (!e) e |= dev_alloc(tx, &tx->d_nfrags, 4);
+    if (resident_only) {
+        auto up = [](uint64_t v) { return (v + 255u) & ~255ull; };
+        const uint64_t o_seq = up(text_bytes), o_qual = o_seq + up(8ull * max_records), o_len = o_qual + up(8ull * max_records);
+        const uint64_t o_reads = o_len + up(4ull * max_records), o_nf = o_reads + up((uint64_t)max_records * sizeof(tgsf_read_result));
+        uint8_t* slab = nullptr;
+        e |= dev_alloc(tx, &slab, o_nf + 256);
+        if (!e) {
+            tx->d_text = slab;
+            tx->d_index.seq_off = (uint64_t*)(slab + o_seq);
+            tx->d_index.qual_off = (uint64_t*)(slab + o_qual);
+            tx->d_index.len = (uint32_t*)(slab + o_len);
+            tx->d_reads = (tgsf_read_result*)(slab + o_reads);
+            tx->d_nfrags = (uint32_t*)(slab + o_nf);
+        }
+    } else {
+        e |= dev_alloc(tx, &tx->d_text, text_bytes);
+        if (!e) e |= dev_alloc(tx, &tx->d_bits, tx->max_pieces * kTextPieceWords);
+        if (!e) e |= dev_alloc(tx, &tx->d_cnt, tx->max_pieces + 1);
+        if (!e) e |= dev_alloc(tx, &tx->d_part, tx->max_pieces / kTextScanTile + 2);
+        if (!e) e |= dev_alloc(tx, &tx->d_table, 4ull * max_records);
+        if (!e) e |= dev_alloc(tx, &tx->d_state, 1);
+        if (!e) e |= dev_alloc(tx, &tx->d_index.seq_off, max_records);
+        if (!e) e |= dev_alloc(tx, &tx->d_index.qual_off, max_records);
+        if (!e) e |= dev_alloc(tx, &tx->d_index.len, max_records);
+        if (!e) e |= dev_alloc(tx, &tx->d_index.name_off, max_records);
+        if (!e) e |= dev_alloc(tx, &tx->d_index.name_len, max_records);
+        if (!e) e |= dev_alloc(tx, &tx->d_summary, 1);
+        if (!e) e |= dev_alloc(tx, &tx->d_reads, max_records);
+        if (!e) e |= dev_alloc(tx, &tx->d_nfrags, 4);
+    }
     if (e) {
         tgsf_text_destroy(tx);
         return fail(nullptr, TGSF_E_HIP, "device allocation failed (%llu bytes of text, %u records)", (unsigned long long)max_bytes, max_records);
     }
     *out = tx;
     return TGSF_OK;
+}
+
+extern "C" int tgsf_text_create(int device, uint64_t max_bytes, uint32_t max_records, tgsf_text** out)
+{
+    return create(device, max_bytes, max_records, false, out);
+}
+
+extern "C" int tgsf_text_create_resident(int device, uint64_t max_bytes, uint32_t max_records, tgsf_text** out)
+{
+    return create(device, max_bytes, max_records, true, out);
 }
 
 extern "C" int tgsf_text_profile(tgsf_text* tx, int enable)
@@ -204,6 +245,7 @@
 
 static int check_args(tgsf_text* tx, uint64_t n_bytes, int fasta, int final)
 {
+    if (tx->resident_only) return fail(tx, TGSF_E_INVALID, "the object was made by tgsf_text_create_resident: it has no indexer");
     if ((fasta != 0 && fasta != 1) || (final != 0 && final != 1)) return fail(tx, TGSF_E_INVALID, "fasta and final are 0 or 1");
     if (n_bytes > tx->max_bytes)
         return fail(tx, TGSF_E_CAPACITY, "text of %llu bytes, the indexer was created for %llu", (unsigned long long)n_bytes, (unsigned long long)tx->max_bytes);
@@ -273,6 +315,7 @@
 extern "C" int tgsf_text_fetch(tgsf_text* tx, const tgsf_text_index_arrays* out_index, tgsf_text_summary* out_summary)
 {
     if (!tx) return TGSF_E_INVALID;
+    if (tx->resident_only) return fail(tx, TGSF_E_INVALID, "the object was made by tgsf_text_create_resident: it has no indexer");
 #if !defined(TGSF_EMUL)
     (void)hipSetDevice(tx->device);
 #endif
@@ -296,59 +339,154 @@
     return fetch(tx, out_index, out_summary, &sum);
 }
 
-extern "C" int tgsf_text_submit(tgsf_text* tx, tgsf_ctx* ctx, const uint8_t* text, uint64_t n_bytes, int fasta, int final,
-                                const tgsf_text_index_arrays* out_index, tgsf_text_summary* out_summary, tgsf_batch_out* bo)
-{
-    if (!tx) return TGSF_E_INVALID;
-    if (!ctx || !out_summary || !bo || !bo->reads || (!text && n_bytes)) return fail(tx, TGSF_E_INVALID, "null argument");
-    int e = check_args(tx, n_bytes, fasta, final);
-    if (e) return e;
-#if !defined(TGSF_EMUL)
-    (void)hipSetDevice(tx->device);
-#endif
+static int filter_device(tgsf_text* tx, tgsf_ctx* ctx, uint64_t n_bytes, uint32_t n_records, tgsf_batch_out* bo)
+{
+    bo->n_frags = 0;
+    if (!n_records) return TGSF_OK;
     if (bo->frags && bo->frag_capacity > tx->frag_cap) {
         tgsf_fragment* f = nullptr;
         if (dev_alloc(tx, &f, bo->frag_capacity)) return fail(tx, TGSF_E_HIP, "device allocation failed (%u fragment records)", bo->frag_capacity);
         tx->d_frags = f;
         tx->frag_cap = bo->frag_capacity;
     }
+    tgsf_batch_in in;
+    memset(&in, 0, sizeof in);
+    in.seq = tx->d_text;
+    in.qual = tx->d_text;
+    in.offsets = tx->d_index.seq_off;
+    in.lengths = tx->d_index.len;
+    in.qual_offsets = tx->d_index.qual_off;
+    in.n_reads = n_records;
+    in.n_bytes = n_bytes;
+    tgsf_batch_out dout;
+    dout.reads = tx->d_reads;
+    dout.frags = bo->frags ? tx->d_frags : nullptr;
+    dout.frag_capacity = bo->frags ? bo->frag_capacity : 0u;
+    dout.n_frags = 0;
+    int e = tgsf_submit_device(ctx, &in, &dout, tx->d_nfrags, (void*)tx->stream);
+    if (!e) e = tgsf_wait(ctx);
+    if (e) return fail(tx, e, "libtgsf: %s", tgsf_last_error(ctx));
+    uint32_t nf = 0;
+    int he = rt_d2h(&nf, tx->d_nfrags, 4, tx->stream);
+    he |= rt_d2h(bo->reads, tx->d_reads, (size_t)n_records * sizeof(tgsf_read_result), tx->stream);
+    if (!he) he = rt_sync(tx->stream);
+    if (!he && nf > dout.frag_capacity) return fail(tx, TGSF_E_CAPACITY, "batch produced %u fragments, caller provided room for %u", nf, dout.frag_capacity);
+    if (!he && nf) {
+        he = rt_d2h(bo->frags, tx->d_frags, (size_t)nf * sizeof(tgsf_fragment), tx->stream);
+        if (!he) he = rt_sync(tx->stream);
+    }
+    if (he) return fail(tx, TGSF_E_HIP, "device to host copy failed: %s", rt_errstr(he));
+    bo->n_frags = nf;
+    return TGSF_OK;
+}
+
+extern "C" int tgsf_text_submit(tgsf_text* tx, tgsf_ctx* ctx, const uint8_t* text, uint64_t n_bytes, int fasta, int final,
+                                const tgsf_text_index_arrays* out_index, tgsf_text_summary* out_summary, tgsf_batch_out* bo)
+{
+    if (!tx) return TGSF_E_INVALID;
+    if (!ctx || !out_summary || !bo || !bo->reads || (!text && n_bytes)) return fail(tx, TGSF_E_INVALID, "null argument");
+    int e = check_args(tx, n_bytes, fasta, final);
+    if (e) return e;
+#if !defined(TGSF_EMUL)
+    (void)hipSetDevice(tx->device);
+#endif
     if ((e = upload(tx, text, n_bytes))) return e;
     if ((e = enqueue_index(tx, tx->d_text, n_bytes, fasta, final, tx->d_index, tx->d_summary, tx->stream))) return e;
     tgsf_text_summary sum;
     if ((e = fetch(tx, nullptr, nullptr, &sum))) return e;
-    bo->n_frags = 0;
-    if (sum.n_records) {
-        tgsf_batch_in in;
-        memset(&in, 0, sizeof in);
-        in.seq = tx->d_text;
-        in.qual = tx->d_text;
-        in.offsets = tx->d_index.seq_off;
-        in.lengths = tx->d_index.len;
-        in.qual_offsets = tx->d_index.qual_off;
-        in.n_reads = sum.n_records;
-        in.n_bytes = n_bytes;
-        tgsf_batch_out dout;
-        dout.reads = tx->d_reads;
-        dout.frags = bo->frags ? tx->d_frags : nullptr;
-        dout.frag_capacity = bo->frags ? bo->frag_capacity : 0u;
-        dout.n_frags = 0;
-        e = tgsf_submit_device(ctx, &in, &dout, tx->d_nfrags, (void*)tx->stream);
-        if (!e) e = tgsf_wait(ctx);
-        if (e) return fail(tx, e, "libtgsf: %s", tgsf_last_error(ctx));
-        uint32_t nf = 0;
-        int he = rt_d2h(&nf, tx->d_nfrags, 4, tx->stream);
-        he |= rt_d2h(bo->reads, tx->d_reads, (size_t)sum.n_records * sizeof(tgsf_read_result), tx->stream);
-        if (!he) he = rt_sync(tx->stream);
-        if (!he && nf > dout.frag_capacity) return fail(tx, TGSF_E_CAPACITY, "batch produced %u fragments, caller provided room for %u", nf, dout.frag_capacity);
-        if (!he && nf) {
-            he = rt_d2h(bo->frags, tx->d_frags, (size_t)nf * sizeof(tgsf_fragment), tx->stream);
-            if (!he) he = rt_sync(tx->stream);
-        }
-        if (he) return fail(tx, TGSF_E_HIP, "device to host copy failed: %s", rt_errstr(he));
-        bo->n_frags = nf;
-    }
+    if ((e = filter_device(tx, ctx, n_bytes, sum.n_records, bo))) return e;
     tgsf_text_summary again;
     if (out_index && (e = fetch(tx, out_index, nullptr, &again))) return e;
     *out_summary = sum;
     return TGSF_OK;
 }
+
+
+#if !defined(TGSF_EMUL)
+static size_t stage_piece_bytes()
+{
+    size_t v = 32u << 20;
+    if (const char* e = knob("TGSF_TEXT_STAGE_BYTES")) { const long long k = atoll(e); if (k >= 64 && k <= (1ll << 30)) v = (size_t)k; }
+    return v;
+}
+
+static int staged_h2d(tgsf_text* tx, tgsf_text* via, const uint8_t* text, uint64_t n)
+{
+    if (!via->stage[0]) {
+        via->stage_bytes = stage_piece_bytes();
+        (void)hipSetDevice(via->device);
+        for (int i = 0; i < 2; i++)
+            if (hipHostMalloc((void**)&via->stage[i], via->stage_bytes, hipHostMallocDefault) != hipSuccess || hipEventCreateWithFlags(&via->stage_ev[i], hipEventDisableTiming) != hipSuccess) {
+                (void)hipGetLastError();
+                for (int j = 0; j < 2; j++) {
+                    if (via->stage[j]) { (void)hipHostFree(via->stage[j]); via->stage[j] = nullptr; }
+                    if (via->stage_ev[j]) { (void)hipEventDestroy(via->stage_ev[j]); via->stage_ev[j] = nullptr; }
+                }
+                return fail(tx, TGSF_E_HIP, "pinned staging buffers (2 x %llu bytes) could not be allocated", (unsigned long long)via->stage_bytes);
+            }
+    }
+    int he = 0, k = 0;
+    for (uint64_t o = 0; o < n; o += via->stage_bytes, k ^= 1) {
+        const size_t m = (size_t)std::min<uint64_t>(via->stage_bytes, n - o);
+        (void)hipEventSynchronize(via->stage_ev[k]);
+        memcpy(via->stage[k], text + o, m);
+        he |= (int)hipMemcpyAsync(tx->d_text + o, via->stage[k], m, hipMemcpyHostToDevice, tx->stream);
+        he |= (int)hipEventRecord(via->stage_ev[k], tx->stream);
+    }
+    return he ? fail(tx, TGSF_E_HIP, "host to device copy failed: %s", rt_errstr(he)) : TGSF_OK;
+}
+#endif
+
+extern "C" int tgsf_text_upload_batch(tgsf_text* tx, tgsf_text* via, const uint8_t* text, uint64_t n_bytes,
+                                      const uint64_t* seq_off, const uint64_t* qual_off, const uint32_t* len, uint32_t n_records)
+{
+    if (!tx) return TGSF_E_INVALID;
+    tx->res_bytes = 0; tx->res_records = 0;
+    if ((!text && n_bytes) || (n_records && (!seq_off || !qual_off || !len))) return fail(tx, TGSF_E_INVALID, "null argument");
+    if (n_bytes > tx->max_bytes)
+        return fail(tx, TGSF_E_CAPACITY, "text of %llu bytes, the object was created for %llu", (unsigned long long)n_bytes, (unsigned long long)tx->max_bytes);
+    if (n_records > tx->max_records) return fail(tx, TGSF_E_CAPACITY, "%u records, the object was created for %u", n_records, tx->max_records);
+    if (!via) via = tx;
+    if (via->device != tx->device) return fail(tx, TGSF_E_INVALID, "the staging object lives on another device");
+    int e = TGSF_OK;
+#if !defined(TGSF_EMUL)
+    (void)hipSetDevice(tx->device);
+    if (n_bytes) e = staged_h2d(tx, via, text, n_bytes);
+#else
+    if (n_bytes) e = rt_h2d(tx->d_text, text, n_bytes, tx->stream) ? fail(tx, TGSF_E_HIP, "host to device copy failed") : TGSF_OK;
+#endif
+    if (e) return e;
+    int he = rt_memset(tx->d_text + n_bytes, 0, (size_t)((((n_bytes + 15u) & ~15ull) - n_bytes) + TGSF_TEXT_PAD), tx->stream);
+    if (n_records) {
+        he |= rt_h2d(tx->d_index.seq_off, seq_off, (size_t)n_records * 8, tx->stream);
+        he |= rt_h2d(tx->d_index.qual_off, qual_off, (size_t)n_records * 8, tx->stream);
+        he |= rt_h2d(tx->d_index.len, len, (size_t)n_records * 4, tx->stream);
+    }
+    if (!he) he = rt_sync(tx->stream);
+    if (he) return fail(tx, TGSF_E_HIP, "host to device copy failed: %s", rt_errstr(he));
+    tx->res_bytes = n_bytes; tx->res_records = n_records;
+    return TGSF_OK;
+}
+
+extern "C" int tgsf_text_filter_resident(tgsf_text* tx, tgsf_ctx* ctx, tgsf_batch_out* bo)
+{
+    if (!tx) return TGSF_E_INVALID;
+    if (!ctx || !bo || !bo->reads) return fail(tx, TGSF_E_INVALID, "null argument");
+#if !defined(TGSF_EMUL)
+    (void)hipSetDevice(tx->device);
+#endif
+    return filter_device(tx, ctx, tx->res_bytes, tx->res_records, bo);
+}
+
+extern "C" int tgsf_text_device_memory(int device, uint64_t* free_bytes, uint64_t* total_bytes)
+{
+    size_t f = (size_t)64 << 30, t = (size_t)64 << 30;
+#if !defined(TGSF_EMUL)
+    if (hipSetDevice(device) != hipSuccess) return fail(nullptr, TGSF_E_NO_DEVICE, "hipSetDevice(%d) failed: no usable HIP device (there is no CPU fallback)", device);
+    if (hipMemGetInfo(&f, &t) != hipSuccess) { (void)hipGetLastError(); return fail(nullptr, TGSF_E_HIP, "hipMemGetInfo failed"); }
+#endif
+    (void)device;
+    if (free_bytes) *free_bytes = f;
+    if (total_bytes) *total_bytes = t;
+    return TGSF_OK;
+}
diff --git a/tgsfilter_amd/host/api.cpp b/tgsfilter_amd/host/api.cpp
--- a/tgsfilter_amd/host/api.cpp
+++ b/tgsfilter_amd/host/api.cpp
@@ -9,6 +9,7 @@
 #include <cstdio>
 #include <cstdlib>
 #include <iostream>
+#include <mutex>
 #include <string>
 #include <thread>
 
@@ -23,6 +24,7 @@
 
 namespace {
 Api g_api;
+TextApi g_text;
 std::thread g_thread;
 std::string g_error;
 double g_load_s = 0, g_device_s = 0;
@@ -79,6 +81,35 @@
             return;
         }
     }
+    {
+        const size_t slash = path.rfind('/');
+        const size_t base = slash == std::string::npos ? 0 : slash + 1;
+        std::string tpath = path;
+        if (path.compare(base, 7, "libtgsf") == 0) tpath.insert(base + 7, "_text");
+        else tpath = path.substr(0, base) + "libtgsf_text.so";
+        void* ht = dlopen(tpath.c_str(), RTLD_NOW | RTLD_LOCAL);
+        if (!ht) { g_error = std::string("cannot load ") + tpath + ": " + dlerror() + " (there is no CPU fallback)"; return; }
+#define BIND(field, sym) \
+    g_text.field = reinterpret_cast<decltype(g_text.field)>(dlsym(ht, sym)); \
+    if (!g_text.field) { g_error = std::string("symbol ") + sym + " missing in " + tpath; return; }
+        BIND(abi_version, "tgsf_text_abi_version")
+        BIND(backend, "tgsf_text_backend")
+        BIND(create_resident, "tgsf_text_create_resident")
+        BIND(destroy, "tgsf_text_destroy")
+        BIND(last_error, "tgsf_text_last_error")
+        BIND(upload_batch, "tgsf_text_upload_batch")
+        BIND(filter_resident, "tgsf_text_filter_resident")
+        BIND(device_memory, "tgsf_text_device_memory")
+#undef BIND
+        if (g_text.abi_version() != TGSF_TEXT_ABI_VERSION) { g_error = tpath + ": ABI version mismatch"; return; }
+        const char* b = g_text.backend();
+        const std::string want = TGSF_EXPECT_BACKEND;
+        if (!b || std::string(b).compare(0, want.size(), want) != 0) {
+            g_error = tpath + " is the \"" + (b ? b : "?") + "\" build of the library; this program runs on the \"" + want +
+                      "\" build only (there is no CPU fallback; is TGSF_LIB set by accident?)";
+            return;
+        }
+    }
     g_load_s = now_s() - t0;
     std::vector<std::thread> up;
     for (size_t i = 1; i < devices.size(); i++) {
@@ -100,13 +131,22 @@
 
 const Api& lib()
 {
-    if (!g_started) lib_start({});
-    if (g_thread.joinable()) g_thread.join();
+    static std::once_flag joined;
+    std::call_once(joined, [] {
+        if (!g_started) lib_start({});
+        if (g_thread.joinable()) g_thread.join();
+    });
     if (!g_error.empty()) {
         std::cerr << "Error: " << g_error << std::endl;
         quit(255);
     }
     return g_api;
+}
+
+const TextApi& text_lib()
+{
+    (void)lib();
+    return g_text;
 }
 
 namespace {
diff --git a/tgsfilter_amd/host/api.h b/tgsfilter_amd/host/api.h
--- a/tgsfilter_amd/host/api.h
+++ b/tgsfilter_amd/host/api.h
@@ -3,6 +3,7 @@
 
 #include "tgsf.h"
 #include "tgsf_rccl.h"
+#include "tgsf_text.h"
 
 namespace host {
 
@@ -26,6 +27,17 @@
     decltype(&tgsf_counters_merge) counters_merge;
 };
 
+struct TextApi {
+    decltype(&tgsf_text_abi_version) abi_version;
+    decltype(&tgsf_text_backend) backend;
+    decltype(&tgsf_text_create_resident) create_resident;
+    decltype(&tgsf_text_destroy) destroy;
+    decltype(&tgsf_text_last_error) last_error;
+    decltype(&tgsf_text_upload_batch) upload_batch;
+    decltype(&tgsf_text_filter_resident) filter_resident;
+    decltype(&tgsf_text_device_memory) device_memory;
+};
+
 struct RcclApi {
     decltype(&tgsf_rccl_unique_id) unique_id;
     decltype(&tgsf_rccl_comm_init) comm_init;
@@ -39,6 +51,7 @@
 
 void lib_start(const std::vector<int>& devices);
 const Api& lib();
+const TextApi& text_lib();
 void lib_times(double& load_s, double& device_s);
 
 }
diff --git a/tgsfilter_amd/host/main.cpp b/tgsfilter_amd/host/main.cpp
--- a/tgsfilter_amd/host/main.cpp
+++ b/tgsfilter_amd/host/main.cpp
@@ -125,6 +125,7 @@
     if (const int rc = run.check_file_types()) return rc;
     run.open_input();
     run.open_output_early();
+    run.plan_batches();
     run.prepass();
     run.make_contexts();
     run.filter_pass();
diff --git a/tgsfilter_amd/host/pipeline.h b/tgsfilter_amd/host/pipeline.h
--- a/tgsfilter_amd/host/pipeline.h
+++ b/tgsfilter_amd/host/pipeline.h
@@ -31,6 +31,7 @@
 #include "fastx.h"
 #include "options.h"
 #include "tgsf.h"
+#include "tgsf_text.h"
 #include "textsource.h"
 
 namespace host {
@@ -60,7 +61,10 @@
     char* dst = nullptr;
     uint64_t out_bytes = 0;
     std::atomic<int> left{0};
+    tgsf_text* slot = nullptr;
+    bool slot_once = false;
     void reset() {
+        slot = nullptr; slot_once = false;
         base = nullptr; span = 0; off.clear(); qoff.clear(); len.clear(); recs.clear(); n_frags = 0; bases = 0; id = 0;
         em.clear(); hold.reset(); dst = nullptr; out_bytes = 0; left = 0;
     }
diff --git a/tgsfilter_amd/host/run.h b/tgsfilter_amd/host/run.h
--- a/tgsfilter_amd/host/run.h
+++ b/tgsfilter_amd/host/run.h
@@ -20,6 +20,7 @@
     int check_file_types();
     void open_input();
     void open_output_early();
+    void plan_batches();
     void prepass();
     void make_contexts();
     void filter_pass();
@@ -90,7 +91,28 @@
     bool mapped_out = false;
     void reader_body();
     void feed(size_t k);
-    void bind_to_node_of(size_t k);
+    void bind_to_node_of(size_t k, bool record = true);
+    std::vector<std::unique_ptr<Channel<std::shared_ptr<Batch>>>> resident;
+    std::thread reader_t;
+    std::vector<std::thread> uploaders;
+    bool early_started = false, early_started_ahead = false;
+    void start_upload();
+    void upload_body(size_t k);
+    tgsf_text* take_slot(size_t k, uint64_t need, bool& once);
+    void return_slot(size_t k, tgsf_text* s, bool once);
+    struct SlotRing {
+        std::mutex m;
+        std::condition_variable cv;
+        std::vector<tgsf_text*> free;
+        size_t n_slots = 0, n_uploaders = 0;
+        uint64_t slot_bytes = 0, budget = 0;
+        bool budget_known = false, grow = true, ctx_ready = false;
+        double waited = 0, t_first_h2d = 0, t_last_h2d = 0;
+        uint64_t uploaded = 0, resident_at_ctx = 0;
+    };
+    std::vector<std::unique_ptr<SlotRing>> rings;
+    std::vector<size_t> ctx_di;
+    std::atomic<int> numa_known{0};
     void writer_body();
     void fill_job(const std::shared_ptr<Batch>& b, size_t lo, size_t hi);
     void batch_done(std::shared_ptr<Batch> b);
diff --git a/tgsfilter_amd/host/run_contexts.cpp b/tgsfilter_amd/host/run_contexts.cpp
--- a/tgsfilter_amd/host/run_contexts.cpp
+++ b/tgsfilter_amd/host/run_contexts.cpp
@@ -2,8 +2,65 @@
 
 namespace host {
 
+static uint32_t reads_per_batch(const Options& o, const std::vector<size_t>& adapter_lens, size_t n_adapters)
+{
+    uint32_t batch_reads = 1u << 16;
+    uint64_t per_read = 0, cols = 0, words = 1;
+    for (const size_t alen : adapter_lens) {
+        const int Q = (int)alen;
+        const int kmax = std::max(0, std::min(Q - 1, std::max(Q - o.end_match_len + 1, Q - o.mid_match_len + 1)));
+        cols = std::max<uint64_t>(cols, (uint64_t)(Q + kmax + 2));
+        words = std::max<uint64_t>(words, Q > 256 ? (uint64_t)(Q + 63) / 64 : Q > 128 ? 4 : Q > 64 ? 2 : 1);
+    }
+    per_read = cols * 2 * words * 8;
+    if (words > 4) per_read = std::min<uint64_t>(per_read, (1ull << 20) + 16 * words) + 32 * words + 512;
+    per_read *= 3 * std::max<size_t>(n_adapters, 1);
+    if (per_read) batch_reads = (uint32_t)std::min<uint64_t>(batch_reads, std::max<uint64_t>(256, (4ull << 30) / per_read));
+    return batch_reads;
+}
+
+void Run::plan_batches()
+{
+    batch_text = streaming ? std::min<uint64_t>(256ull << 20, chunk_bytes)
+                                    : std::min<uint64_t>(256ull << 20, std::max<uint64_t>(text_size / 8 + 4096, 1 << 16));
+    if (const char* e = knob("TGSF_BATCH_BYTES")) { const long long v = atoll(e); if (v > 0) batch_text = (uint64_t)v; }
+    std::vector<size_t> lens;
+    size_t n = 0;
+    if (o.filter && !o.adapter_file.empty()) {
+        auto add = [&](const std::string& a) { if (std::find(adapters.begin(), adapters.end(), a) == adapters.end()) adapters.push_back(a); };
+        InputBytes af;
+        if (af.open(o.adapter_file)) {
+            const int ft = file_type(o.adapter_file);
+            FastxReader rd(af.data(), af.size(), ft == 1);
+            Record r;
+            while (rd.next(r)) { add(std::string(r.seq)); add(rev_comp(std::string(r.seq))); }
+        }
+        for (const std::string& a : adapters) lens.push_back(a.size());
+        n = adapters.size();
+    } else if (o.filter) {
+        size_t longest = 0;
+        for (const char* a : kAdapterLib) longest = std::max(longest, strlen(a));
+        lens.push_back(longest);
+        n = 4;
+    }
+    batch_reads = reads_per_batch(o, lens, n);
+    fastq_out = o.out_type == 1;
+    run_filter_pass = o.filter || o.only_qc;
+    int per_dev = (streaming || text_size > (64u << 20)) ? 3 : 1;
+    if (const char* e = getenv("TGSF_CTX_PER_DEVICE")) { const int v = atoi(e); if (v >= 1 && v <= 8) per_dev = v; }
+    for (size_t di = 0; di < o.devices.size(); di++) for (int k = 0; k < per_dev; k++) { ctx_dev.push_back(o.devices[di]); ctx_di.push_back(di); }
+    ctxs.assign(ctx_dev.size(), nullptr);
+    dev_node.assign(ctx_dev.size(), -1);
+    dev_submit_s.assign(ctx_dev.size(), 0.0);
+    dev_bytes.assign(ctx_dev.size(), 0);
+    dev_batches.assign(ctx_dev.size(), 0);
+    const char* ahead = getenv("TGSF_AHEAD_BYTES");
+    if (!streaming && run_filter_pass && !(ahead && strtoull(ahead, nullptr, 10) == 0)) { early_started_ahead = true; start_upload(); }
+}
+
 void Run::prepass()
 {
+    if (const char* e = knob("TGSF_PREPASS_HOLD_S")) usleep((useconds_t)(atof(e) * 1e6));
     std::unique_ptr<CpuScope> cpu_prepass(new CpuScope(CPU_PREPASS));
     if (sharded && link.rank > 0) {
     } else if (streaming) {
@@ -49,13 +106,6 @@
         if (!fasta_in) std::cerr << "INFO: min Phred average quality score: " << o.min_q << std::endl;
         auto add = [&](const std::string& a) { if (std::find(adapters.begin(), adapters.end(), a) == adapters.end()) adapters.push_back(a); };
         if (!o.adapter_file.empty()) {
-            InputBytes af;
-            if (af.open(o.adapter_file)) {
-                const int ft = file_type(o.adapter_file);
-                FastxReader rd(af.data(), af.size(), ft == 1);
-                Record r;
-                while (rd.next(r)) { add(std::string(r.seq)); add(rev_comp(std::string(r.seq))); }
-            }
             int num = 0;
             for (const std::string& a : adapters) std::cerr << "INFO: input adapter " << ++num << " :" << a << std::endl;
         } else {
@@ -84,25 +134,6 @@
 
 void Run::make_contexts()
 {
-    batch_text = streaming ? std::min<uint64_t>(256ull << 20, chunk_bytes)
-                                    : std::min<uint64_t>(256ull << 20, std::max<uint64_t>(text_size / 8 + 4096, 1 << 16));
-    if (const char* e = knob("TGSF_BATCH_BYTES")) { const long long v = atoll(e); if (v > 0) batch_text = (uint64_t)v; }
-    batch_reads = 1u << 16;
-    {
-        uint64_t per_read = 0, cols = 0, words = 1;
-        for (const std::string& a : adapters) {
-            const int Q = (int)a.size();
-            const int kmax = std::max(0, std::min(Q - 1, std::max(Q - o.end_match_len + 1, Q - o.mid_match_len + 1)));
-            cols = std::max<uint64_t>(cols, (uint64_t)(Q + kmax + 2));
-            words = std::max<uint64_t>(words, Q > 256 ? (uint64_t)(Q + 63) / 64 : Q > 128 ? 4 : Q > 64 ? 2 : 1);
-        }
-        per_read = cols * 2 * words * 8;
-        if (words > 4) per_read = std::min<uint64_t>(per_read, (1ull << 20) + 16 * words) + 32 * words + 512;
-        per_read *= 3 * std::max<size_t>(adapters.size(), 1);
-        if (per_read) batch_reads = (uint32_t)std::min<uint64_t>(batch_reads, std::max<uint64_t>(256, (4ull << 30) / per_read));
-    }
-    fastq_out = o.out_type == 1;
-    run_filter_pass = o.filter || o.only_qc;
     {
         const bool may_map = plain_file_out() && !o.only_qc && !o.downsample && run_filter_pass;
         if (may_map && !mapped.is_open()) mapped.open(out_path, streaming ? std::max<uint64_t>(64ull << 30, 64ull * in.size())
@@ -176,10 +207,6 @@
     else if (records_p->complete()) p.max_read_len = std::max<uint32_t>(records_p->longest(), 1024);
     else p.max_read_len = (uint32_t)std::min<uint64_t>(std::max<uint64_t>(in.size() / 2, 1024), 1u << 26);
     p.max_batch_bases = std::max<uint64_t>(batch_text, 2ull * p.max_read_len + (1u << 16)) + (1 << 20);
-    int per_dev = (streaming || text_size > (64u << 20)) ? 3 : 1;
-    if (const char* e = getenv("TGSF_CTX_PER_DEVICE")) { const int v = atoi(e); if (v >= 1 && v <= 8) per_dev = v; }
-    for (int d : o.devices) for (int k = 0; k < per_dev; k++) ctx_dev.push_back(d);
-    ctxs.assign(ctx_dev.size(), nullptr);
     t_p0 = now_s();
 }
 
diff --git a/tgsfilter_amd/host/run_pipeline.cpp b/tgsfilter_amd/host/run_pipeline.cpp
--- a/tgsfilter_amd/host/run_pipeline.cpp
+++ b/tgsfilter_amd/host/run_pipeline.cpp
@@ -7,7 +7,7 @@
 void Run::reader_body()
 {
     CpuScope cpu(CPU_BATCHER);
-    if (!run_filter_pass) { for (size_t d = 0; d < ctxs.size(); d++) to_gpu->put(nullptr); return; }
+    if (!run_filter_pass) { for (size_t d = 0; d < ctx_dev.size(); d++) to_gpu->put(nullptr); return; }
     std::unique_ptr<RecordIndex::Cursor> rd;
     if (!streaming) rd.reset(new RecordIndex::Cursor(*records_p));
     std::unique_ptr<ChunkReader> cr;
@@ -52,7 +52,6 @@
     const char* last_end = nullptr;
     while (next_record()) {
         const size_t L = r.len;
-        if (L > p.max_read_len) die("read longer than the supported maximum");
         const char* rec_end = (fasta_in ? r.seq : r.qual) + L;
         if (sharded && !last_end && link.rank > 0 && r.name != text + 1) bad_cut(text_off);
         last_end = rec_end;
@@ -62,7 +61,6 @@
         b->qoff.push_back(fasta_in ? b->off.back() : (uint64_t)(r.qual - b->base));
         b->len.push_back((uint32_t)L); b->recs.push_back(r);
         b->span = (uint64_t)(rec_end - b->base);
-        if (b->span > p.max_batch_bases) die("record larger than a batch");
         b->bases += L;
         raw_bases += L; raw_lens.push_back((int)L);
     }
@@ -74,12 +72,12 @@
         if (e != end || !records_p->end_message().empty()) bad_cut(text_off + text_size);
     }
     flush();
-    for (size_t d = 0; d < ctxs.size(); d++) to_gpu->put(nullptr);
+    for (size_t d = 0; d < ctx_dev.size(); d++) to_gpu->put(nullptr);
     t_parse = now_s() - t0 - waited;
     std::sort(raw_lens.begin(), raw_lens.end());
 }
 
-void Run::bind_to_node_of(size_t k)
+void Run::bind_to_node_of(size_t k, bool record)
 {
     const Api& L = *api;
     int node = -1;
@@ -110,33 +108,138 @@
                 if (CPU_ISSET(c2, &set)) n_set++;
             }
         }
-        if (n_set > 0 && sched_setaffinity(0, sizeof set, &set) == 0) dev_node[k] = node;
-    }
+        if (n_set > 0 && sched_setaffinity(0, sizeof set, &set) == 0 && record) dev_node[k] = node;
+    }
+}
+
+tgsf_text* Run::take_slot(size_t k, uint64_t need, bool& once)
+{
+    const TextApi& T = text_lib();
+    SlotRing& ring = *rings[ctx_di[k]];
+    const int device = ctx_dev[k];
+    auto make = [&](uint64_t bytes) {
+        tgsf_text* tx = nullptr;
+        return T.create_resident(device, bytes, batch_reads, &tx) == TGSF_OK ? tx : nullptr;
+    };
+    once = need > ring.slot_bytes;
+    if (once) {
+        tgsf_text* tx = make(need);
+        if (!tx) die(T.last_error(nullptr));
+        return tx;
+    }
+    std::unique_lock<std::mutex> l(ring.m);
+    if (!ring.budget_known) {
+        uint64_t free_b = 0;
+        ring.budget = std::min<uint64_t>((uint64_t)text_size / rings.size() + ring.slot_bytes, 32ull << 30);
+        if (T.device_memory(device, &free_b, nullptr) == TGSF_OK) ring.budget = std::min(ring.budget, free_b / 2);
+        if (const char* e = getenv("TGSF_AHEAD_BYTES")) ring.budget = strtoull(e, nullptr, 10);
+        ring.budget_known = true;
+    }
+    const size_t floor_slots = 2 * ring.n_uploaders;
+    double w0 = 0;
+    for (;;) {
+        if (!ring.free.empty()) { tgsf_text* tx = ring.free.back(); ring.free.pop_back(); if (w0 != 0) ring.waited += now_s() - w0; return tx; }
+        if (ring.grow && (ring.n_slots < floor_slots || (!ring.ctx_ready && (ring.n_slots + 1) * ring.slot_bytes <= ring.budget))) {
+            ring.n_slots++;
+            l.unlock();
+            tgsf_text* tx = make(ring.slot_bytes);
+            l.lock();
+            if (tx) { if (w0 != 0) ring.waited += now_s() - w0; return tx; }
+            ring.n_slots--;
+            ring.grow = false;
+            if (ring.n_slots == 0) die(T.last_error(nullptr));
+            continue;
+        }
+        if (w0 == 0) w0 = now_s();
+        ring.cv.wait(l);
+    }
+}
+
+void Run::return_slot(size_t k, tgsf_text* s, bool once)
+{
+    if (once) { text_lib().destroy(s); return; }
+    SlotRing& ring = *rings[ctx_di[k]];
+    { std::lock_guard<std::mutex> l(ring.m); ring.free.push_back(s); }
+    ring.cv.notify_one();
+}
+
+void Run::upload_body(size_t k)
+{
+    CpuScope cpu(CPU_FEEDER);
+    const TextApi& T = text_lib();
+    SlotRing& ring = *rings[ctx_di[k]];
+    bool bound = false;
+    auto bind = [&] { if (!bound && numa_known.load(std::memory_order_acquire)) { bound = true; if (numa_bind) bind_to_node_of(k, false); } };
+    tgsf_text* via = nullptr;
+    if (T.create_resident(ctx_dev[k], 16, 1, &via) != TGSF_OK) die(T.last_error(nullptr));
+    for (;;) {
+        std::shared_ptr<Batch> b = to_gpu->get();
+        if (!b) break;
+        bind();
+        bool once = false;
+        tgsf_text* slot = take_slot(k, b->span, once);
+        const double u0 = now_s();
+        if (T.upload_batch(slot, via, reinterpret_cast<const uint8_t*>(b->base), b->span, b->off.data(), b->qoff.data(), b->len.data(),
+                           (uint32_t)b->recs.size()) != TGSF_OK) die(T.last_error(slot));
+        {
+            std::lock_guard<std::mutex> l(ring.m);
+            if (ring.t_first_h2d == 0) ring.t_first_h2d = u0 - t_start;
+            ring.t_last_h2d = now_s() - t_start;
+            ring.uploaded += b->span;
+        }
+        b->slot = slot; b->slot_once = once;
+        resident[ctx_di[k]]->put(std::move(b));
+    }
+    resident[ctx_di[k]]->put(nullptr);
+}
+
+void Run::start_upload()
+{
+    to_gpu.reset(new Channel<std::shared_ptr<Batch>>(2 + ctx_dev.size()));
+    for (size_t k = 0; k < ctx_dev.size(); k++) {
+        if (ctx_di[k] == rings.size()) {
+            rings.emplace_back(new SlotRing);
+            resident.emplace_back(new Channel<std::shared_ptr<Batch>>(1u << 20));
+            rings.back()->slot_bytes = batch_text;
+        }
+        rings[ctx_di[k]]->n_uploaders++;
+    }
+    early_started = true;
+    reader_t = std::thread([this] { reader_body(); });
+    for (size_t k = 0; k < ctx_dev.size(); k++) uploaders.emplace_back([this, k] { upload_body(k); });
 }
 
 void Run::feed(size_t k)
 {
     CpuScope cpu(CPU_FEEDER);
     const Api& L = *api;
+    const TextApi& T = text_lib();
     if (numa_bind) bind_to_node_of(k);
     if (L.create(&p, ctx_dev[k], &ctxs[k]) != TGSF_OK) die(L.last_error(nullptr));
     tgsf_ctx* fctx = ctxs[k];
+    SlotRing& ring = *rings[ctx_di[k]];
+    {
+        std::lock_guard<std::mutex> l(ring.m);
+        if (!ring.ctx_ready) { ring.ctx_ready = true; ring.resident_at_ctx = ring.uploaded; }
+    }
     if (timing) (void)L.profile(fctx, 1);
     for (;;) {
-        std::shared_ptr<Batch> b = to_gpu->get();
+        std::shared_ptr<Batch> b = resident[ctx_di[k]]->get();
         if (!b) break;
         const double g0 = now_s();
+        for (const uint32_t len : b->len) if (len > p.max_read_len) die("read longer than the supported maximum");
+        if (b->span > p.max_batch_bases) die("record larger than a batch");
         if (b->res.size() < b->recs.size()) b->res.resize(b->recs.size());
         const size_t fneed = (size_t)(b->bases / (uint64_t)std::max(p.min_len, 1)) + b->recs.size() + 16;
         if (b->frags.size() < fneed) b->frags.resize(fneed);
-        const uint8_t* btext = reinterpret_cast<const uint8_t*>(b->base);
-        tgsf_batch_in bi;
-        memset(&bi, 0, sizeof bi);
-        bi.seq = btext; bi.qual = btext;
-        bi.offsets = b->off.data(); bi.qual_offsets = b->qoff.data(); bi.lengths = b->len.data();
-        bi.n_reads = (uint32_t)b->recs.size(); bi.n_bytes = b->span;
         tgsf_batch_out bo{b->res.data(), b->frags.data(), (uint32_t)b->frags.size(), 0};
-        if (L.submit(fctx, &bi, &bo) != TGSF_OK) die(L.last_error(fctx));
+        if (T.filter_resident(b->slot, fctx, &bo) != TGSF_OK) {
+            std::string msg = T.last_error(b->slot);
+            if (msg.compare(0, 9, "libtgsf: ") == 0) msg.erase(0, 9);
+            die(msg);
+        }
+        return_slot(k, b->slot, b->slot_once);
+        b->slot = nullptr;
         { std::lock_guard<std::mutex> l(gpu_time_m); t_gpu += now_s() - g0; if (t_first == 0) t_first = now_s() - t_p0; }
         dev_submit_s[k] += now_s() - g0; dev_bytes[k] += b->span; dev_batches[k]++;
         b->n_frags = bo.n_frags;
@@ -154,7 +257,6 @@
 
 void Run::filter_pass()
 {
-    to_gpu.reset(new Channel<std::shared_ptr<Batch>>(2 + ctxs.size()));
     to_writer.reset(new Channel<std::shared_ptr<Batch>>(256));
     if (!run_filter_pass) {
         RecordIndex::Cursor rd(*records_p);
@@ -165,14 +267,11 @@
         }
     }
 
-    std::thread reader([this] { reader_body(); });
+    if (!early_started) start_upload();
 
     numa_bind = o.devices.size() > 1 || (link.world > 1 && ranks_own_gpus);
     if (const char* e = getenv("TGSF_NUMA")) numa_bind = atoi(e) > 0;
-    dev_node.assign(ctx_dev.size(), -1);
-    dev_submit_s.assign(ctx_dev.size(), 0.0);
-    dev_bytes.assign(ctx_dev.size(), 0);
-    dev_batches.assign(ctx_dev.size(), 0);
+    numa_known.store(1, std::memory_order_release);
     std::vector<std::thread> feeders;
     for (size_t k = 0; k < ctxs.size(); k++) feeders.emplace_back([this, k] { feed(k); });
 
@@ -198,7 +297,8 @@
     release_output = sync_exit || streaming;
     mapped.start_filling(fill_threads, 16u << 20);
     std::thread writer([this] { writer_body(); });
-    reader.join();
+    reader_t.join();
+    for (std::thread& u : uploaders) u.join();
     for (std::thread& f : feeders) f.join();
     writer.join();
     mapped_out = mapped.is_open();
diff --git a/tgsfilter_amd/host/run_report.cpp b/tgsfilter_amd/host/run_report.cpp
--- a/tgsfilter_amd/host/run_report.cpp
+++ b/tgsfilter_amd/host/run_report.cpp
@@ -279,6 +279,21 @@
                         "first batch filtered after %.3f, fill tail %.3f, closing the output %.3f; stages overlap) | stats+report %.3f | %s (fallocate %.3f, mapping the reserved pages %.3f, fill threads busy %.3f summed)\n",
                 now_s() - t_start, t_prepass, t_libwait, t_load, t_dev, t_pipe, t_parse, ctxs.size(), t_gpu, t_write, t_widle, t_first,
                 mapped.t_fill_tail, mapped.t_close, now_s() - t_p0 - t_pipe, mapped_out ? "output: fallocate + mapped fill" : "output: writev", mapped.sink.t_falloc, mapped.t_populate_wait(), t_busy);
+        {
+            double first = 0, last = 0, waited = 0;
+            uint64_t at_ctx = 0, up = 0;
+            size_t slots = 0;
+            for (const std::unique_ptr<SlotRing>& r : rings) {
+                if (r->t_first_h2d > 0 && (first == 0 || r->t_first_h2d < first)) first = r->t_first_h2d;
+                last = std::max(last, r->t_last_h2d); waited += r->waited; at_ctx += r->resident_at_ctx; up += r->uploaded; slots += r->n_slots;
+            }
+            char who[48] = "";
+            if (sharded) snprintf(who, sizeof who, "DEVICE %d ", o.device);
+            fprintf(stderr, "%sUPLOAD: first H2D at %.3f s, last H2D done at %.3f s (process start = 0) | %llu bytes resident when the first context was ready, "
+                            "%llu uploaded | %zu slots of %llu bytes | uploaders waited %.3f s for a slot | started %s\n",
+                    who, first, last, (unsigned long long)at_ctx, (unsigned long long)up, slots, (unsigned long long)batch_text, waited,
+                    early_started_ahead ? "ahead of the pre-pass" : "behind the pre-pass");
+        }
         fprintf(stderr, "RESERVE: planner waited %.3f s for pages of the output file\n", mapped.t_claim_wait);
     }
     if (timing) {
diff --git a/tgsfilter_amd/text.py b/tgsfilter_amd/text.py
--- a/tgsfilter_amd/text.py
+++ b/tgsfilter_amd/text.py
@@ -13,7 +13,7 @@
 DEFAULT_LIB = os.path.join(_HERE, "libtgsf_text.so")
 _LIBS = {}
 
-ABI_VERSION = 1
+ABI_VERSION = 2
 END, IRREGULAR, CAPACITY = 0, 1, 2
 STOP_NAMES = {END: "END", IRREGULAR: "IRREGULAR", CAPACITY: "CAPACITY"}
 PAD = 64
@@ -21,6 +21,7 @@
 SYMBOLS = [
     "tgsf_text_abi_version", "tgsf_text_backend", "tgsf_text_create", "tgsf_text_destroy", "tgsf_text_last_error", "tgsf_text_profile",
     "tgsf_text_buffers", "tgsf_text_index", "tgsf_text_upload", "tgsf_text_index_device", "tgsf_text_fetch", "tgsf_text_submit",
+    "tgsf_text_create_resident", "tgsf_text_upload_batch", "tgsf_text_filter_resident", "tgsf_text_device_memory",
 ]
 
 
@@ -70,6 +71,10 @@
         L.tgsf_text_index_device.argtypes = [vp, vp, u64, i, i, C.POINTER(IndexArrays), vp, vp]
         L.tgsf_text_fetch.argtypes = [vp, C.POINTER(IndexArrays), C.POINTER(Summary)]
         L.tgsf_text_submit.argtypes = [vp, vp, vp, u64, i, i, C.POINTER(IndexArrays), C.POINTER(Summary), C.POINTER(abi.BatchOut)]
+        L.tgsf_text_create_resident.argtypes = [i, u64, C.c_uint32, C.POINTER(vp)]
+        L.tgsf_text_upload_batch.argtypes = [vp, vp, vp, u64, vp, vp, vp, C.c_uint32]
+        L.tgsf_text_filter_resident.argtypes = [vp, vp, C.POINTER(abi.BatchOut)]
+        L.tgsf_text_device_memory.argtypes = [i, C.POINTER(u64), C.POINTER(u64)]
         if L.tgsf_text_abi_version() != ABI_VERSION:
             raise RuntimeError("libtgsf_text ABI version mismatch")
         _LIBS[path] = L
@@ -87,11 +92,12 @@
 
 class TextIndexer:
 
-    def __init__(self, device: int, max_bytes: int, max_records: int, lib_path: str | None = None):
+    def __init__(self, device: int, max_bytes: int, max_records: int, lib_path: str | None = None, resident_only: bool = False):
         self.lib = load(lib_path)
         self.max_bytes, self.max_records = int(max_bytes), int(max_records)
         h = C.c_void_p()
-        rc = self.lib.tgsf_text_create(device, self.max_bytes, self.max_records, C.byref(h))
+        make = self.lib.tgsf_text_create_resident if resident_only else self.lib.tgsf_text_create
+        rc = make(device, self.max_bytes, self.max_records, C.byref(h))
         if rc != 0:
             raise TgsfError(rc, self.lib.tgsf_text_last_error(None).decode())
         self.h = h
@@ -166,3 +172,21 @@
                                             C.byref(ia) if want_index else None, C.byref(s), C.byref(bo)))
         n = s.n_records
         return (self._clip(arrs, n) if want_index else None), s.as_dict(), reads[:n].copy(), frags[:bo.n_frags].copy()
+
+    def upload_batch(self, text, seq_off, qual_off, lengths, via: "TextIndexer | None" = None):
+        t = _as_u8(text)
+        so = np.ascontiguousarray(seq_off, dtype=np.uint64)
+        qo = np.ascontiguousarray(qual_off, dtype=np.uint64)
+        ln = np.ascontiguousarray(lengths, dtype=np.uint32)
+        assert so.size == qo.size == ln.size
+        self._resident_records = int(so.size)
+        self._chk(self.lib.tgsf_text_upload_batch(self.h, via.h if via is not None else None, t.ctypes.data, t.size,
+                                                  so.ctypes.data, qo.ctypes.data, ln.ctypes.data, so.size))
+
+    def filter_resident(self, ctx, frag_capacity):
+        n = self._resident_records
+        reads = np.zeros(max(n, 1), dtype=abi.READ_RESULT_DTYPE)
+        frags = np.zeros(frag_capacity, dtype=abi.FRAGMENT_DTYPE)
+        bo = abi.BatchOut(reads.ctypes.data, frags.ctypes.data, frag_capacity, 0)
+        self._chk(self.lib.tgsf_text_filter_resident(self.h, ctx.h, C.byref(bo)))
+        return reads[:n].copy(), frags[:bo.n_frags].copy()
```

Result: slower. 5.467 (-20.2%).
